# haoheliu/AudioLDM2

Hardware: AMD Instinct MI355X
Metric: audio_seconds_per_second (higher is better)
Workload: dtype f32 storage/accumulate; each product = 6 bf16 MFMA partial products of exact 3-part operand splits (fp32-grade); 1 GPU; audioldm2-full: batch 8 prompts/GPU x 1 GPU, 10.24 s @16 kHz, 200 DDIM steps, CFG 3.5, eta 1.0, n_candidates 1; one step = sample_log + VAE decode + HiFi-GAN + D2H of the waveform; synthetic conditioning, random-init weights, host-CPU RNG noise; global_batch=8, parallelism=prompt-sharded replicas x1, weight_broadcast_bytes=0

## Files before the change

audioldm2_amd/csrc/api.hip:

```cpp
#include "common.h"
#include <string.h>

namespace aldm {
static thread_local char g_err[512] = "";
void set_error(const char* fmt, ...) {
    va_list ap;
    va_start(ap, fmt);
    vsnprintf(g_err, sizeof(g_err), fmt, ap);
    va_end(ap);
}
}

extern "C" int aldm_version(void) { return 11; }
extern "C" const char* aldm_last_error(void) { return aldm::g_err; }
```

audioldm2_amd/csrc/norm.hip:

```cpp
#include <stdlib.h>
#include "igemm_epilogue.h"

namespace aldm {

constexpr int GN_ITERS = 16;
constexpr int GN_UNROLL = 8;

struct GnPart {
    float n, mean, m2;
};

__device__ __forceinline__ void gn_merge(double& n, double& mean, double& m2, double nb, double mb, double m2b) {
    if (nb <= 0.0) return;
    const double nt = n + nb;
    const double dlt = mb - mean;
    mean += dlt * (nb / nt);
    m2 += m2b + dlt * dlt * (n * nb / nt);
    n = nt;
}

template <bool FUSED>
__global__ __launch_bounds__(256) void gn_partial_kernel(const float* __restrict__ x1,
                                                         const float* __restrict__ x2, int P,
                                                         int C1, int C2, int G, int cols, int rows,
                                                         int chunk_px, float* __restrict__ ws, float eps,
                                                         const float* __restrict__ gamma,
                                                         const float* __restrict__ beta,
                                                         float* __restrict__ scale, float* __restrict__ shift, int gpb,
                                                         char* __restrict__ dst = nullptr, char* __restrict__ dst_raw = nullptr,
                                                         int parts = 3, int act = ALDM_ACT_NONE, int raw_parts = 3,
                                                         float f16_scale = 0.f) {
    const int C = C1 + C2;
    const int Cg4 = (C / G) >> 2;
    const int b = blockIdx.y;
    const int chunk = FUSED ? 0 : blockIdx.x;
    const int g_lo = FUSED ? blockIdx.x * gpb : 0;
    const int c4_lo = g_lo * Cg4, C4 = c4_lo + gpb * Cg4;
    const int p0 = chunk * chunk_px;
    const int p1 = min(P, p0 + chunk_px);
    const int tid = threadIdx.x;
    const int tx = tid % cols, ty = tid / cols;
    __shared__ GnPart ps[256];
    const int npass = (C4 - c4_lo + cols - 1) / cols;
    __shared__ double gacc[64][3];
    if (tid < 64) gacc[tid][0] = gacc[tid][1] = gacc[tid][2] = 0.0;
    __syncthreads();
    for (int cp = 0; cp < npass; ++cp) {
        const int c4 = c4_lo + cp * cols + tx;
        GnPart part = {0.f, 0.f, 0.f};
        if (ty < rows && c4 < C4 && p0 + ty < p1) {
            const int c = c4 << 2;
            const bool first = c < C1;
            const float* src = first ? x1 + (int64_t)b * P * C1 + c : x2 + (int64_t)b * P * C2 + (c - C1);
            const int pitch = first ? C1 : C2;
            float sa[GN_UNROLL], sq[GN_UNROLL];
#pragma unroll
            for (int u = 0; u < GN_UNROLL; ++u) sa[u] = sq[u] = 0.f;
            int p = p0 + ty;
            const float pivot = src[(int64_t)p * pitch];
            int cnt = 0;
            for (; p + (GN_UNROLL - 1) * rows < p1; p += GN_UNROLL * rows) {
                f32x4 v[GN_UNROLL];
#pragma unroll
                for (int u = 0; u < GN_UNROLL; ++u)
                    v[u] = *reinterpret_cast<const f32x4*>(src + (int64_t)(p + u * rows) * pitch) - pivot;
#pragma unroll
                for (int u = 0; u < GN_UNROLL; ++u) {
                    sa[u] += (v[u][0] + v[u][1]) + (v[u][2] + v[u][3]);
                    sq[u] += (v[u][0] * v[u][0] + v[u][1] * v[u][1]) + (v[u][2] * v[u][2] + v[u][3] * v[u][3]);
                }
                cnt += GN_UNROLL;
            }
            for (; p < p1; p += rows) {
                const f32x4 v = *reinterpret_cast<const f32x4*>(src + (int64_t)p * pitch) - pivot;
                sa[0] += (v[0] + v[1]) + (v[2] + v[3]);
                sq[0] += (v[0] * v[0] + v[1] * v[1]) + (v[2] * v[2] + v[3] * v[3]);
                ++cnt;
            }
            float s = 0.f, ss = 0.f;
#pragma unroll
            for (int u = 0; u < GN_UNROLL; u += 2) {
                s += sa[u] + sa[u + 1];
                ss += sq[u] + sq[u + 1];
            }
            const float n = 4.0f * (float)cnt;
            const float md = s / n;
            part.n = n;
            part.mean = pivot + md;
            part.m2 = fmaxf(ss - s * md, 0.f);
        }
        if constexpr (FUSED) {
            __shared__ double wred[4][3];
            const int mygl = (c4 - c4_lo) / Cg4;
            for (int gl = 0; gl < gpb; ++gl) {
                const bool mine = part.n > 0.f && mygl == gl;
                double n = mine ? (double)part.n : 0.0, mean = mine ? (double)part.mean : 0.0, m2 = mine ? (double)part.m2 : 0.0;
#pragma unroll
                for (int o = 32; o > 0; o >>= 1) {
                    const double nb = __shfl_xor(n, o), mb = __shfl_xor(mean, o), m2b = __shfl_xor(m2, o);
                    gn_merge(n, mean, m2, nb, mb, m2b);
                }
                if ((tid & 63) == 0) {
                    wred[tid >> 6][0] = n;
                    wred[tid >> 6][1] = mean;
                    wred[tid >> 6][2] = m2;
                }
                __syncthreads();
                if (tid == 0) {
                    double an = gacc[gl][0], am = gacc[gl][1], a2 = gacc[gl][2];
                    for (int w = 0; w < 4; ++w) gn_merge(an, am, a2, wred[w][0], wred[w][1], wred[w][2]);
                    gacc[gl][0] = an;
                    gacc[gl][1] = am;
                    gacc[gl][2] = a2;
                }
                __syncthreads();
            }
            continue;
        }
        ps[tid] = part;
        __syncthreads();
        if (tid < gpb) {
            const int g = g_lo + tid;
            const int base = c4_lo + cp * cols;
            const int lo = max(g * Cg4, base), hi = min((g + 1) * Cg4, min(C4, base + cols));
            if (lo < hi) {
                double n = gacc[tid][0], mean = gacc[tid][1], m2 = gacc[tid][2];
                for (int yy = 0; yy < rows; ++yy)
                    for (int cc = lo; cc < hi; ++cc) {
                        const GnPart& t = ps[yy * cols + (cc - base)];
                        gn_merge(n, mean, m2, (double)t.n, (double)t.mean, (double)t.m2);
                    }
                gacc[tid][0] = n;
                gacc[tid][1] = mean;
                gacc[tid][2] = m2;
            }
        }
        __syncthreads();
    }
    if (FUSED) {
        const int Cg = C / G;
        __shared__ float fin[64][2];
        if (tid < gpb) {
            const double n = gacc[tid][0];
            double var = n > 0.0 ? gacc[tid][2] / n : 0.0;
            if (var < 0.0) var = 0.0;
            fin[tid][0] = (float)gacc[tid][1];
            fin[tid][1] = (float)(1.0 / sqrt(var + (double)eps));
        }
        __syncthreads();
        __shared__ float lsc[256], lsh[256];
        for (int c = g_lo * Cg + tid; c < (g_lo + gpb) * Cg; c += 256) {
            const int g = c / Cg - g_lo;
            const float sc = fin[g][1] * (gamma ? gamma[c] : 1.f);
            const float sh = (beta ? beta[c] : 0.f) - fin[g][0] * sc;
            scale[(int64_t)b * C + c] = sc;
            shift[(int64_t)b * C + c] = sh;
            if (dst) {
                lsc[c - g_lo * Cg] = sc;
                lsh[c - g_lo * Cg] = sh;
            }
        }
        if (dst) {
            __syncthreads();
            const int c_lo = g_lo * Cg, sw = (gpb * Cg) >> 3;
            for (int i = tid; i < P * sw; i += 256) {
                const int p = i / sw;
                const int cl = (i - p * sw) << 3;
                const int c = c_lo + cl;
                const int64_t row = (int64_t)b * P + p;
                const float* src = c < C1 ? x1 + row * C1 + c : x2 + row * C2 + (c - C1);
                f32x4 v0 = *reinterpret_cast<const f32x4*>(src);
                f32x4 v1 = *reinterpret_cast<const f32x4*>(src + 4);
                const int64_t off = (row * (C >> 5) + (c >> 5)) * (64 * parts) + (c & 31) * 2;
                u32x2 p0[3], p1[3];
                if (dst_raw) {
                    const int64_t roff = (row * (C >> 5) + (c >> 5)) * (64 * raw_parts) + (c & 31) * 2;
                    split4_parts(v0, p0, raw_parts);
                    split4_parts(v1, p1, raw_parts);
#pragma unroll
                    for (int q = 0; q < 3; ++q)
                        if (q < raw_parts)
                            *reinterpret_cast<u32x4*>(dst_raw + roff + q * 64) = u32x4{p0[q][0], p0[q][1], p1[q][0], p1[q][1]};
                }
#pragma unroll
                for (int e = 0; e < 4; ++e) {
                    v0[e] = __builtin_fmaf(v0[e], lsc[cl + e], lsh[cl + e]);
                    v1[e] = __builtin_fmaf(v1[e], lsc[cl + 4 + e], lsh[cl + 4 + e]);
                }
                if (act == ALDM_ACT_SILU) {
#pragma unroll
                    for (int e = 0; e < 4; ++e) {
                        v0[e] = silu_fast(v0[e]);
                        v1[e] = silu_fast(v1[e]);
                    }
                }
                split4_fmt(v0, p0, parts, f16_scale);
                split4_fmt(v1, p1, parts, f16_scale);
#pragma unroll
                for (int q = 0; q < 3; ++q)
                    if (q < parts) *reinterpret_cast<u32x4*>(dst + off + q * 64) = u32x4{p0[q][0], p0[q][1], p1[q][0], p1[q][1]};
            }
        }
    } else if (tid < G) {
        double* w = reinterpret_cast<double*>(ws) + ((int64_t)(b * gridDim.x + chunk) * G + tid) * 3;
        w[0] = gacc[tid][0];
        w[1] = gacc[tid][1];
        w[2] = gacc[tid][2];
    }
}

__global__ __launch_bounds__(256) void gn_finalize_kernel(const float* __restrict__ ws, int chunks,
                                                          int P, int C, int G, float eps,
                                                          const float* __restrict__ gamma,
                                                          const float* __restrict__ beta,
                                                          float* __restrict__ scale,
                                                          float* __restrict__ shift) {
    const int b = blockIdx.x;
    __shared__ float s_mean[64], s_rstd[64];
    __shared__ double s_part[256][3];
    const int Cg = C / G;
    const double* wsd = reinterpret_cast<const double*>(ws);
    const int LPG = 256 / G >= 1 ? 256 / G : 1;
    {
        const int g = threadIdx.x / LPG, l = threadIdx.x % LPG;
        double n = 0.0, mean = 0.0, m2 = 0.0;
        if (g < G) {
            for (int ch = l; ch < chunks; ch += LPG) {
                const double* w = wsd + ((int64_t)(b * chunks + ch) * G + g) * 3;
                gn_merge(n, mean, m2, w[0], w[1], w[2]);
            }
        }
        s_part[threadIdx.x][0] = n;
        s_part[threadIdx.x][1] = mean;
        s_part[threadIdx.x][2] = m2;
    }
    __syncthreads();
    if (threadIdx.x < G) {
        const int g = threadIdx.x;
        double n = 0.0, mean = 0.0, m2 = 0.0;
        for (int l = 0; l < LPG; ++l) gn_merge(n, mean, m2, s_part[g * LPG + l][0], s_part[g * LPG + l][1], s_part[g * LPG + l][2]);
        double var = n > 0.0 ? m2 / n : 0.0;
        if (var < 0.0) var = 0.0;
        s_mean[g] = (float)mean;
        s_rstd[g] = (float)(1.0 / sqrt(var + (double)eps));
    }
    __syncthreads();
    for (int c = threadIdx.x; c < C; c += blockDim.x) {
        const int g = c / Cg;
        const float ga = gamma ? gamma[c] : 1.f;
        const float be = beta ? beta[c] : 0.f;
        const float sc = s_rstd[g] * ga;
        scale[(int64_t)b * C + c] = sc;
        shift[(int64_t)b * C + c] = be - s_mean[g] * sc;
    }
}

constexpr int LN_MAXV = 8;

template <int MAXV, int R, bool RMS = false>
__global__ __launch_bounds__(256) void layernorm_kernel(const float* __restrict__ x,
                                                        float* __restrict__ y, int M, int C,
                                                        const float* __restrict__ gamma,
                                                        const float* __restrict__ beta, float eps,
                                                        void* __restrict__ y_split, int parts, float f16_scale) {
    const int lane = threadIdx.x & 63;
    const int row0 = (blockIdx.x * 4 + (threadIdx.x >> 6)) * R;
    if (row0 >= M) return;
    const int C4 = C >> 2;
    f32x4 v[R][MAXV];
#pragma unroll
    for (int r = 0; r < R; ++r) {
        const float* xr = x + (int64_t)min(row0 + r, M - 1) * C;
#pragma unroll
        for (int i = 0; i < MAXV; ++i) {
            const int c4 = lane + 64 * i;
            v[r][i] = c4 < C4 ? *reinterpret_cast<const f32x4*>(xr + 4 * c4) : f32x4{0.f, 0.f, 0.f, 0.f};
        }
    }
    f32x4 ga[MAXV], be[MAXV];
#pragma unroll
    for (int i = 0; i < MAXV; ++i) {
        const int c4 = min(lane + 64 * i, C4 - 1);
        ga[i] = *reinterpret_cast<const f32x4*>(gamma + 4 * c4);
        be[i] = RMS ? f32x4{0.f, 0.f, 0.f, 0.f} : *reinterpret_cast<const f32x4*>(beta + 4 * c4);
    }
    float mean[R], rstd[R];
#pragma unroll
    for (int r = 0; r < R; ++r) {
        float s = 0.f;
#pragma unroll
        for (int i = 0; i < MAXV; ++i) s += (v[r][i][0] + v[r][i][1]) + (v[r][i][2] + v[r][i][3]);
#pragma unroll
        for (int o = 32; o > 0; o >>= 1) s += __shfl_xor(s, o);
        mean[r] = RMS ? 0.f : s / (float)C;
    }
#pragma unroll
    for (int r = 0; r < R; ++r) {
        float q = 0.f;
#pragma unroll
        for (int i = 0; i < MAXV; ++i) {
            if (lane + 64 * i < C4) {
                const f32x4 dlt = v[r][i] - mean[r];
                q += (dlt[0] * dlt[0] + dlt[1] * dlt[1]) + (dlt[2] * dlt[2] + dlt[3] * dlt[3]);
            }
        }
#pragma unroll
        for (int o = 32; o > 0; o >>= 1) q += __shfl_xor(q, o);
        rstd[r] = 1.0f / sqrtf(q / (float)C + eps);
    }
#pragma unroll
    for (int r = 0; r < R; ++r) {
        if (row0 + r >= M) break;
        float* yr = y ? y + (int64_t)(row0 + r) * C : nullptr;
#pragma unroll
        for (int i = 0; i < MAXV; ++i) {
            const int c4 = lane + 64 * i;
            if (c4 < C4) {
                const f32x4 o = (v[r][i] - mean[r]) * rstd[r] * ga[i] + be[i];
                if (yr) *reinterpret_cast<f32x4*>(yr + 4 * c4) = o;
                if (y_split) {
                    if (f16_scale != 0.f) {
                        u32x2 part[3];
                        split4_f16(o, f16_scale, part);
                        char* base = reinterpret_cast<char*>(y_split) + ((int64_t)(row0 + r) * (C >> 5) + (c4 >> 3)) * 128 + (c4 & 7) * 8;
                        *reinterpret_cast<u32x2*>(base) = part[0];
                        *reinterpret_cast<u32x2*>(base + 64) = part[1];
                    } else {
                        split_store4(y_split, row0 + r, C, 4 * c4, o, parts);
                    }
                }
            }
        }
    }
}

template <bool MASKED, bool BIASED = false>
__global__ __launch_bounds__(256) void softmax_rows_kernel(const float* __restrict__ x,
                                                           float* __restrict__ y, int N,
                                                           float scale, const float* __restrict__ keymask,
                                                           int rows_per_batch, int q_rows, int q_pos0,
                                                           const float* __restrict__ bias = nullptr) {
    extern __shared__ __attribute__((aligned(16))) float srow[];
    __shared__ float red[4];
    const int64_t row = blockIdx.x;
    const float* xr = x + row * N;
    float* yr = y + row * N;
    const int tid = threadIdx.x;
    float mx = -INFINITY;
    const float* km = nullptr;
    int jmax = N;
    const float* br = nullptr;
    if (MASKED) {
        km = keymask + (row / rows_per_batch) * N;
        jmax = BIASED ? N : q_pos0 + (int)(row % q_rows) + 1;
    }
    if (BIASED) br = bias + (row % rows_per_batch) * N;
    for (int i = tid; i < N; i += 256) {
        float v = xr[i] * scale;
        if (BIASED) v += br[i];
        if (MASKED && (i >= jmax || km[i] == 0.0f)) v = -INFINITY;
        srow[i] = v;
        mx = fmaxf(mx, v);
    }
#pragma unroll
    for (int o = 32; o > 0; o >>= 1) mx = fmaxf(mx, __shfl_xor(mx, o));
    if ((tid & 63) == 0) red[tid >> 6] = mx;
    __syncthreads();
    mx = fmaxf(fmaxf(red[0], red[1]), fmaxf(red[2], red[3]));
    __syncthreads();
    float s = 0.f;
    for (int i = tid; i < N; i += 256) {
        const float e = (MASKED && srow[i] == -INFINITY) ? 0.0f : expf(srow[i] - mx);
        srow[i] = e;
        s += e;
    }
#pragma unroll
    for (int o = 32; o > 0; o >>= 1) s += __shfl_xor(s, o);
    if ((tid & 63) == 0) red[tid >> 6] = s;
    __syncthreads();
    s = (red[0] + red[1]) + (red[2] + red[3]);
    const float inv = 1.0f / s;
    for (int i = tid; i < N; i += 256) yr[i] = srow[i] * inv;
}

static void gn_geometry(int P, int C, int* cols, int* rows, int* chunk_px, int* chunks) {
    const int C4 = C / 4;
    *cols = C4 < 256 ? C4 : 256;
    *rows = 256 / *cols;
    if (*rows < 1) *rows = 1;
    *chunk_px = *rows * GN_ITERS;
    *chunks = (P + *chunk_px - 1) / *chunk_px;
}

}

using namespace aldm;

extern "C" int64_t aldm_gn_ws_floats(int B, int P, int C, int G) {
    int cols, rows, chunk_px, chunks;
    gn_geometry(P, C, &cols, &rows, &chunk_px, &chunks);
    return (int64_t)B * chunks * G * 6 + 2;
}

extern "C" int aldm_split_rows(const float* x1, const float* x2, int C1, int C2, int64_t rows, int P, const float* scale,
                               const float* shift, int act, void* dst, void* dst_raw, int parts, void* stream);
extern "C" int aldm_split_rows_f16(const float* x1, const float* x2, int C1, int C2, int64_t rows, int P, const float* scale,
                                   const float* shift, int act, float slope, void* dst, void* dst_raw, int raw_parts, float f16_scale,
                                   void* stream);

static int groupnorm_launch(const float* x1, const float* x2, int B, int P, int C1, int C2, int G, float eps,
                            const float* gamma, const float* beta, float* scale, float* shift, float* ws, void* dst,
                            void* dst_raw, int parts, int act, void* stream, int raw_parts = 0, float f16_scale = 0.f) {
    if (raw_parts == 0) raw_parts = parts;
    if (!x2) C2 = 0;
    const int C = C1 + C2;
    ALDM_CHECK(x1 && scale && shift && ws, "aldm_groupnorm_stats: null pointer");
    ws = reinterpret_cast<float*>((reinterpret_cast<uintptr_t>(ws) + 7) & ~uintptr_t(7));
    ALDM_CHECK(G > 0 && G <= 64 && C % G == 0 && (C / G) % 4 == 0 && C1 % 4 == 0,
               "aldm_groupnorm_stats: need C%%G==0, (C/G)%%4==0, C1%%4==0 (C1=%d C2=%d G=%d)", C1, C2, G);
    int cols, rows, chunk_px, chunks;
    gn_geometry(P, C, &cols, &rows, &chunk_px, &chunks);
    hipStream_t st = (hipStream_t)stream;
    static const int64_t fused_max = [] {
        const char* e = getenv("ALDM_GN_FUSED_MAX");
        return e ? (int64_t)atoll(e) : (int64_t)1 << 17;
    }();
    int gs = 1;
    while (gs < G && gs * B < 256 && G % (gs * 2) == 0) gs *= 2;
    const int gpb = G / gs;
    if ((int64_t)P * C <= fused_max && P <= 1024 && gpb <= 4) {
        const int c4b = gpb * (C / G) / 4;
        const int fcols = c4b < 256 ? c4b : 256, frows = 256 / fcols;
        const int slab = gpb * (C / G);
        static const bool fuse_split = [] {
            const char* e = getenv("ALDM_GN_SPLIT_FUSED");
            return e == nullptr || e[0] != '0';
        }();
        if (dst && fuse_split && slab % 8 == 0 && slab <= 256 && C1 % 8 == 0) {
            hipLaunchKernelGGL(gn_partial_kernel<true>, dim3(gs, B), dim3(256), 0, st, x1, x2, P, C1, C2, G, fcols, frows, P, ws,
                               eps, gamma, beta, scale, shift, gpb, reinterpret_cast<char*>(dst),
                               reinterpret_cast<char*>(dst_raw), parts, act, raw_parts, f16_scale);
            ALDM_LAUNCH_CHECK("aldm_groupnorm_split");
            return 0;
        }
        hipLaunchKernelGGL(gn_partial_kernel<true>, dim3(gs, B), dim3(256), 0, st, x1, x2, P, C1, C2, G, fcols,
                           frows, P, ws, eps, gamma, beta, scale, shift, gpb, nullptr, nullptr, 3, ALDM_ACT_NONE);
    } else {
        hipLaunchKernelGGL(gn_partial_kernel<false>, dim3(chunks, B), dim3(256), 0, st, x1, x2, P, C1, C2, G,
                           cols, rows, chunk_px, ws, eps, gamma, beta, scale, shift, G);
        hipLaunchKernelGGL(gn_finalize_kernel, dim3(B), dim3(256), 0, st, ws, chunks, P, C, G, eps, gamma,
                           beta, scale, shift);
    }
    ALDM_LAUNCH_CHECK("aldm_groupnorm_stats");
    if (dst) {
        if (f16_scale != 0.f)
            return aldm_split_rows_f16(x1, x2, C1, C2, (int64_t)B * P, P, scale, shift, act, 0.f, dst, dst_raw, raw_parts, f16_scale, stream);
        return aldm_split_rows(x1, x2, C1, C2, (int64_t)B * P, P, scale, shift, act, dst, dst_raw, parts, stream);
    }
    return 0;
}

extern "C" int aldm_groupnorm_stats(const float* x1, const float* x2, int B, int P, int C1, int C2,
                                    int G, float eps, const float* gamma, const float* beta,
                                    float* scale, float* shift, float* ws, void* stream) {
    return groupnorm_launch(x1, x2, B, P, C1, C2, G, eps, gamma, beta, scale, shift, ws, nullptr, nullptr, 3, ALDM_ACT_NONE,
                            stream);
}

extern "C" int aldm_groupnorm_split(const float* x1, const float* x2, int B, int P, int C1, int C2, int G, float eps,
                                    const float* gamma, const float* beta, int act, float* scale, float* shift, float* ws,
                                    void* dst, void* dst_raw, int parts, void* stream) {
    if (!x2) C2 = 0;
    ALDM_CHECK(dst != nullptr && (parts == 2 || parts == 3) && (C1 + C2) % 32 == 0 && C1 % 8 == 0 && C2 % 8 == 0,
               "aldm_groupnorm_split: need dst, parts 2|3, (C1+C2) %% 32 == 0, C1 %% 8 == 0 (C1=%d C2=%d)", C1, C2);
    ALDM_CHECK(act == ALDM_ACT_NONE || act == ALDM_ACT_SILU, "aldm_groupnorm_split: activation %d not supported", act);
    ALDM_CHECK(((reinterpret_cast<uintptr_t>(dst) | reinterpret_cast<uintptr_t>(dst_raw)) & 15) == 0,
               "aldm_groupnorm_split: split images must be 16-byte aligned");
    return groupnorm_launch(x1, x2, B, P, C1, C2, G, eps, gamma, beta, scale, shift, ws, dst, dst_raw, parts, act, stream);
}

extern "C" int aldm_groupnorm_split_f16(const float* x1, const float* x2, int B, int P, int C1, int C2, int G, float eps,
                                        const float* gamma, const float* beta, int act, float* scale, float* shift, float* ws,
                                        void* dst, void* dst_raw, int raw_parts, float f16_scale, void* stream) {
    if (!x2) C2 = 0;
    ALDM_CHECK(dst != nullptr && f16_scale > 0.0f && (raw_parts == 2 || raw_parts == 3) && (C1 + C2) % 32 == 0 && C1 % 8 == 0 && C2 % 8 == 0,
               "aldm_groupnorm_split_f16: need dst, f16_scale > 0, raw_parts 2|3, (C1+C2) %% 32 == 0, C1 %% 8 == 0 (C1=%d C2=%d)", C1, C2);
    ALDM_CHECK(act == ALDM_ACT_NONE || act == ALDM_ACT_SILU, "aldm_groupnorm_split_f16: activation %d not supported", act);
    ALDM_CHECK(((reinterpret_cast<uintptr_t>(dst) | reinterpret_cast<uintptr_t>(dst_raw)) & 15) == 0,
               "aldm_groupnorm_split_f16: split images must be 16-byte aligned");
    return groupnorm_launch(x1, x2, B, P, C1, C2, G, eps, gamma, beta, scale, shift, ws, dst, dst_raw, 2, act, stream, raw_parts, f16_scale);
}

static int layernorm_launch(const float* x, float* y, void* y_split, int parts, int M, int C, const float* gamma,
                            const float* beta, float eps, void* stream, const char* name, bool rms = false, float f16_scale = 0.f) {
    ALDM_CHECK(parts == 2 || parts == 3, "%s: parts must be 2 or 3", name);
    ALDM_CHECK(x && (y || y_split) && gamma && (beta || rms), "%s: null pointer", name);
    ALDM_CHECK(C % 4 == 0 && C <= 256 * LN_MAXV, "%s: C=%d must be a multiple of 4 and <= %d", name, C, 256 * LN_MAXV);
    ALDM_CHECK(y_split == nullptr || (C % 32 == 0 && (reinterpret_cast<uintptr_t>(y_split) & 15) == 0),
               "%s: a split-image output needs C %% 32 == 0 and 16-byte alignment", name);
    hipStream_t st = (hipStream_t)stream;
#define ALDM_LN(V_, R_)                                                                                             \
    do {                                                                                                            \
        if (rms)                                                                                                    \
            hipLaunchKernelGGL((layernorm_kernel<V_, R_, true>), dim3(cdiv(M, 4 * R_)), dim3(256), 0, st, x, y, M, C, \
                               gamma, beta, eps, y_split, parts, f16_scale);                                        \
        else                                                                                                        \
            hipLaunchKernelGGL((layernorm_kernel<V_, R_, false>), dim3(cdiv(M, 4 * R_)), dim3(256), 0, st, x, y, M, \
                               C, gamma, beta, eps, y_split, parts, f16_scale);                                     \
    } while (0)
    const int nv = cdiv(C / 4, 64);
    static const int env_r = [] {
        const char* e = getenv("ALDM_LN_R");
        return e ? atoi(e) : 0;
    }();
    if (nv <= 1) {
        if (env_r == 4) ALDM_LN(1, 4);
        else if (env_r == 2) ALDM_LN(1, 2);
        else ALDM_LN(1, 1);
    } else if (nv <= 2) {
        if (env_r == 4) ALDM_LN(2, 4);
        else if (env_r == 2) ALDM_LN(2, 2);
        else ALDM_LN(2, 1);
    } else if (nv <= 4) ALDM_LN(4, 2);
    else ALDM_LN(8, 1);
#undef ALDM_LN
    ALDM_LAUNCH_CHECK(name);
    return 0;
}

extern "C" int aldm_layernorm(const float* x, float* y, int M, int C, const float* gamma,
                              const float* beta, float eps, void* stream) {
    return layernorm_launch(x, y, nullptr, 3, M, C, gamma, beta, eps, stream, "aldm_layernorm");
}

extern "C" int aldm_layernorm_split(const float* x, float* y, void* y_split, int M, int C, const float* gamma,
                                    const float* beta, float eps, int parts, void* stream) {
    return layernorm_launch(x, y, y_split, parts, M, C, gamma, beta, eps, stream, "aldm_layernorm_split");
}

extern "C" int aldm_layernorm_split_f16(const float* x, float* y, void* y_split, int M, int C, const float* gamma,
                                        const float* beta, float eps, float f16_scale, void* stream) {
    ALDM_CHECK(y_split != nullptr && f16_scale > 0.0f, "aldm_layernorm_split_f16: need y_split and f16_scale > 0");
    return layernorm_launch(x, y, y_split, 2, M, C, gamma, beta, eps, stream, "aldm_layernorm_split_f16", false, f16_scale);
}

extern "C" int aldm_rmsnorm(const float* x, float* y, int M, int C, const float* weight, float eps, void* stream) {
    return layernorm_launch(x, y, nullptr, 3, M, C, weight, nullptr, eps, stream, "aldm_rmsnorm", true);
}

extern "C" int aldm_softmax_rows(const float* x, float* y, int64_t M, int N, float scale,
                                 void* stream) {
    ALDM_CHECK(x && y && M > 0 && N > 0, "aldm_softmax_rows: bad args");
    ALDM_CHECK((int64_t)N * 4 <= 60 * 1024, "aldm_softmax_rows: row of %d floats exceeds the 60 KiB LDS stage", N);
    ALDM_CHECK(M < (1ll << 31), "aldm_softmax_rows: too many rows");
    hipLaunchKernelGGL(softmax_rows_kernel<false>, dim3((unsigned)M), dim3(256), (size_t)N * 4,
                       (hipStream_t)stream, x, y, N, scale, nullptr, 1, 1, 0);
    ALDM_LAUNCH_CHECK("aldm_softmax_rows");
    return 0;
}

extern "C" int aldm_softmax_rows_masked(const float* x, float* y, int B, int heads, int q_rows, int N, float scale,
                                        const float* keymask, int q_pos0, void* stream) {
    ALDM_CHECK(x && y && keymask && B > 0 && heads > 0 && q_rows > 0 && N > 0 && q_pos0 >= 0,
               "aldm_softmax_rows_masked: bad args");
    ALDM_CHECK((int64_t)N * 4 <= 60 * 1024, "aldm_softmax_rows_masked: row of %d floats exceeds the 60 KiB LDS stage", N);
    const int64_t M = (int64_t)B * heads * q_rows;
    ALDM_CHECK(M < (1ll << 31), "aldm_softmax_rows_masked: too many rows");
    hipLaunchKernelGGL(softmax_rows_kernel<true>, dim3((unsigned)M), dim3(256), (size_t)N * 4, (hipStream_t)stream, x, y,
                       N, scale, keymask, heads * q_rows, q_rows, q_pos0);
    ALDM_LAUNCH_CHECK("aldm_softmax_rows_masked");
    return 0;
}

extern "C" int aldm_softmax_rows_bias(const float* x, float* y, int B, int heads, int q_rows, int N, float scale,
                                      const float* bias, const float* keymask, void* stream) {
    ALDM_CHECK(x && y && bias && keymask && B > 0 && heads > 0 && q_rows > 0 && N > 0, "aldm_softmax_rows_bias: bad args");
    ALDM_CHECK((int64_t)N * 4 <= 60 * 1024, "aldm_softmax_rows_bias: row of %d floats exceeds the 60 KiB LDS stage", N);
    const int64_t M = (int64_t)B * heads * q_rows;
    ALDM_CHECK(M < (1ll << 31), "aldm_softmax_rows_bias: too many rows");
    hipLaunchKernelGGL((softmax_rows_kernel<true, true>), dim3((unsigned)M), dim3(256), (size_t)N * 4, (hipStream_t)stream, x,
                       y, N, scale, keymask, heads * q_rows, q_rows, 0, bias);
    ALDM_LAUNCH_CHECK("aldm_softmax_rows_bias");
    return 0;
}
```

audioldm2_amd/lib.py:

```python
from __future__ import annotations

import ctypes as C
import os

_HERE = os.path.dirname(os.path.abspath(__file__))
LIB_PATH = os.environ.get("ALDM_LIB_PATH") or os.path.join(_HERE, "libaldm_hip.so")
ABI_VERSION = 11

ACT_NONE, ACT_SILU, ACT_LRELU, ACT_TANH, ACT_LOGCLAMP, ACT_GELU, ACT_GELU_TANH = range(7)
B_PACKED, B_NT = 0, 1
EPI_PLAIN, EPI_GEGLU, EPI_QKV = 0, 1, 2
FMT_BF16, FMT_F16 = 0, 1


class IgemmDesc(C.Structure):

    _fields_ = [
        ("x1", C.c_void_p), ("x2", C.c_void_p),
        ("C1", C.c_int32), ("C2", C.c_int32),
        ("pix1", C.c_int32), ("pix2", C.c_int32),
        ("B", C.c_int32), ("H", C.c_int32), ("W", C.c_int32),
        ("up_h", C.c_int32), ("up_w", C.c_int32),
        ("KH", C.c_int32), ("KW", C.c_int32), ("SH", C.c_int32), ("SW", C.c_int32),
        ("PH", C.c_int32), ("PW", C.c_int32), ("DH", C.c_int32), ("DW", C.c_int32),
        ("OH", C.c_int32), ("OW", C.c_int32),
        ("pre_scale", C.c_void_p), ("pre_shift", C.c_void_p),
        ("pre_act", C.c_int32), ("pre_slope", C.c_float),
        ("w", C.c_void_p),
        ("b_mode", C.c_int32), ("ldb", C.c_int32),
        ("K", C.c_int32), ("N", C.c_int32),
        ("bias", C.c_void_p), ("rowbias", C.c_void_p), ("res", C.c_void_p), ("out", C.c_void_p),
        ("ldo", C.c_int32), ("act", C.c_int32), ("act_slope", C.c_float), ("alpha", C.c_float),
        ("accumulate", C.c_int32),
        ("out_mul", C.c_int32), ("out_off", C.c_int32), ("out_len", C.c_int32),
        ("batch", C.c_int32),
        ("stride_x", C.c_int64), ("stride_w", C.c_int64), ("stride_o", C.c_int64),
        ("rowbias_ld", C.c_int32), ("epi_mode", C.c_int32),
        ("ws", C.c_void_p), ("ws_floats", C.c_int64),
        ("hint_bm", C.c_int32), ("hint_bn", C.c_int32), ("hint_splits", C.c_int32), ("hint_kgroups", C.c_int32),
        ("w_split", C.c_void_p), ("hint_mma", C.c_int32), ("hint_stages", C.c_int32),
        ("a_split", C.c_void_p), ("out_split", C.c_void_p), ("out_split_c", C.c_int32), ("split_parts", C.c_int32),
        ("out_split_act", C.c_int32), ("out_split_slope", C.c_float),
        ("k_split", C.c_void_p), ("vt_split", C.c_void_p), ("qkv_c", C.c_int32), ("qkv_rows", C.c_int32),
        ("a_fmt", C.c_int32), ("acc_scale", C.c_float), ("out_split_parts", C.c_int32),
        ("out_split_fmt", C.c_int32), ("out_split_scale", C.c_float), ("vt_scale", C.c_float),
    ]


_SIGS = {
    "aldm_version": (C.c_int, []),
    "aldm_last_error": (C.c_char_p, []),
    "aldm_igemm": (C.c_int, [C.POINTER(IgemmDesc), C.c_void_p]),
    "aldm_igemm_plan": (C.c_int, [C.POINTER(IgemmDesc), C.POINTER(C.c_int), C.POINTER(C.c_int),
                                  C.POINTER(C.c_int64), C.POINTER(C.c_int), C.POINTER(C.c_int),
                                  C.POINTER(C.c_int)]),
    "aldm_igemm_ws_floats": (C.c_int64, [C.POINTER(IgemmDesc)]),
    "aldm_igemm_plan_stages": (C.c_int, [C.POINTER(IgemmDesc)]),
    "aldm_igemm_force": (None, [C.c_int, C.c_int, C.c_int, C.c_int]),
    "aldm_igemm_force_stages": (None, [C.c_int]),
    "aldm_igemm_wave8_mask": (C.c_int, [C.c_int]),
    "aldm_split_image_bytes": (C.c_int64, [C.c_int64, C.c_int, C.c_int]),
    "aldm_split_rows": (C.c_int, [C.c_void_p, C.c_void_p, C.c_int, C.c_int, C.c_int64, C.c_int, C.c_void_p, C.c_void_p,
                                  C.c_int, C.c_void_p, C.c_void_p, C.c_int, C.c_void_p]),
    "aldm_split_rows_act": (C.c_int, [C.c_void_p, C.c_void_p, C.c_int, C.c_int, C.c_int64, C.c_int, C.c_void_p, C.c_void_p,
                                      C.c_int, C.c_float, C.c_void_p, C.c_void_p, C.c_int, C.c_void_p]),
    "aldm_layernorm_split": (C.c_int, [C.c_void_p, C.c_void_p, C.c_void_p, C.c_int, C.c_int, C.c_void_p, C.c_void_p,
                                       C.c_float, C.c_int, C.c_void_p]),
    "aldm_attention_d32_split": (C.c_int, [C.c_void_p, C.c_void_p, C.c_void_p, C.c_void_p, C.c_void_p, C.c_int, C.c_int,
                                           C.c_int, C.c_int, C.c_int, C.c_int, C.c_int, C.c_int, C.c_int,
                                           C.c_void_p, C.c_float, C.c_void_p]),
    "aldm_split_bytes_parts": (C.c_int64, [C.c_int, C.c_int, C.c_int]),
    "aldm_pack_split_bf16_parts": (C.c_int, [C.c_void_p, C.c_void_p, C.c_int, C.c_int, C.c_int, C.c_void_p]),
    "aldm_pack_split_f16": (C.c_int, [C.c_void_p, C.c_void_p, C.c_int, C.c_int, C.c_float, C.c_void_p]),
    "aldm_split_rows_f16": (C.c_int, [C.c_void_p, C.c_void_p, C.c_int, C.c_int, C.c_int64, C.c_int, C.c_void_p, C.c_void_p,
                                      C.c_int, C.c_float, C.c_void_p, C.c_void_p, C.c_int, C.c_float, C.c_void_p]),
    "aldm_groupnorm_split_f16": (C.c_int, [C.c_void_p, C.c_void_p, C.c_int, C.c_int, C.c_int, C.c_int, C.c_int, C.c_float,
                                           C.c_void_p, C.c_void_p, C.c_int, C.c_void_p, C.c_void_p, C.c_void_p, C.c_void_p,
                                           C.c_void_p, C.c_int, C.c_float, C.c_void_p]),
    "aldm_layernorm_split_f16": (C.c_int, [C.c_void_p, C.c_void_p, C.c_void_p, C.c_int, C.c_int, C.c_void_p, C.c_void_p,
                                           C.c_float, C.c_float, C.c_void_p]),
    "aldm_igemm_mma": (C.c_int, [C.c_int]),
    "aldm_split_bytes": (C.c_int64, [C.c_int, C.c_int]),
    "aldm_pack_split_bf16": (C.c_int, [C.c_void_p, C.c_void_p, C.c_int, C.c_int, C.c_void_p]),
    "aldm_pack_weight": (C.c_int, [C.c_void_p, C.c_void_p, C.c_int, C.c_int, C.c_int, C.c_int,
                                   C.c_int, C.c_int, C.c_int, C.c_void_p]),
    "aldm_pack_kn": (C.c_int, [C.c_void_p, C.c_void_p, C.c_int, C.c_int, C.c_int, C.c_int,
                               C.c_int64, C.c_int64, C.c_void_p]),
    "aldm_groupnorm_stats": (C.c_int, [C.c_void_p, C.c_void_p, C.c_int, C.c_int, C.c_int, C.c_int,
                                       C.c_int, C.c_float, C.c_void_p, C.c_void_p, C.c_void_p,
                                       C.c_void_p, C.c_void_p, C.c_void_p]),
    "aldm_gn_ws_floats": (C.c_int64, [C.c_int, C.c_int, C.c_int, C.c_int]),
    "aldm_groupnorm_split": (C.c_int, [C.c_void_p, C.c_void_p, C.c_int, C.c_int, C.c_int, C.c_int, C.c_int, C.c_float,
                                       C.c_void_p, C.c_void_p, C.c_int, C.c_void_p, C.c_void_p, C.c_void_p, C.c_void_p,
                                       C.c_void_p, C.c_int, C.c_void_p]),
    "aldm_layernorm": (C.c_int, [C.c_void_p, C.c_void_p, C.c_int, C.c_int, C.c_void_p, C.c_void_p,
                                 C.c_float, C.c_void_p]),
    "aldm_attention_mma": (C.c_int, [C.c_int]),
    "aldm_attention_sched": (C.c_int, [C.c_int]),
    "aldm_attention_d32_presplit_f16": (C.c_int, [C.c_void_p, C.c_void_p, C.c_void_p, C.c_void_p, C.c_void_p, C.c_int, C.c_float,
                                                  C.c_int, C.c_int, C.c_int, C.c_int, C.c_int, C.c_int, C.c_float, C.c_float,
                                                  C.c_float, C.c_float, C.c_void_p]),
    "aldm_attention_d32_presplit": (C.c_int, [C.c_void_p, C.c_void_p, C.c_void_p, C.c_void_p, C.c_void_p, C.c_int, C.c_int,
                                              C.c_int, C.c_int, C.c_int, C.c_int, C.c_int, C.c_float, C.c_void_p]),
    "aldm_vt_regroup": (C.c_int, [C.c_void_p, C.c_void_p, C.c_int, C.c_int, C.c_int, C.c_int, C.c_void_p]),
    "aldm_attention_d32": (C.c_int, [C.c_void_p, C.c_void_p, C.c_void_p, C.c_void_p, C.c_int,
                                     C.c_int, C.c_int, C.c_int, C.c_int, C.c_int, C.c_int, C.c_int,
                                     C.c_void_p, C.c_float, C.c_void_p]),
    "aldm_rel_attention": (C.c_int, [C.c_void_p, C.c_void_p, C.c_void_p, C.c_void_p, C.c_int, C.c_int, C.c_int, C.c_int,
                                     C.c_int, C.c_int, C.c_int, C.c_int, C.c_void_p, C.c_void_p, C.c_int, C.c_void_p,
                                     C.c_void_p]),
    "aldm_rowscale_add": (C.c_int, [C.c_void_p, C.c_void_p, C.c_void_p, C.c_void_p, C.c_int64, C.c_int, C.c_int, C.c_void_p]),
    "aldm_rmsnorm": (C.c_int, [C.c_void_p, C.c_void_p, C.c_int, C.c_int, C.c_void_p, C.c_float, C.c_void_p]),
    "aldm_softmax_rows_bias": (C.c_int, [C.c_void_p, C.c_void_p, C.c_int, C.c_int, C.c_int, C.c_int, C.c_float, C.c_void_p,
                                         C.c_void_p, C.c_void_p]),
    "aldm_resample_sinc": (C.c_int, [C.c_void_p, C.c_void_p, C.c_void_p, C.c_int, C.c_int, C.c_int, C.c_int, C.c_int, C.c_int,
                                     C.c_int, C.c_void_p]),
    "aldm_power_spec": (C.c_int, [C.c_void_p, C.c_void_p, C.c_int64, C.c_int, C.c_int, C.c_int, C.c_void_p]),
    "aldm_col_affine": (C.c_int, [C.c_void_p, C.c_void_p, C.c_void_p, C.c_void_p, C.c_int64, C.c_int, C.c_void_p]),
    "aldm_bicubic_patchify": (C.c_int, [C.c_void_p, C.c_void_p, C.c_int, C.c_int, C.c_int, C.c_int, C.c_int, C.c_void_p]),
    "aldm_token_mean": (C.c_int, [C.c_void_p, C.c_void_p, C.c_int, C.c_int, C.c_int, C.c_void_p]),
    "aldm_row_cosine": (C.c_int, [C.c_void_p, C.c_void_p, C.c_void_p, C.c_int, C.c_int, C.c_float, C.c_void_p]),
    "aldm_decode_linear": (C.c_int, [C.c_void_p, C.c_int, C.c_int, C.c_int, C.c_void_p, C.c_int, C.c_void_p, C.c_void_p,
                                     C.c_void_p, C.c_float, C.c_int, C.c_void_p, C.c_int, C.c_void_p, C.c_int, C.c_void_p]),
    "aldm_decode_attention": (C.c_int, [C.c_void_p, C.c_int, C.c_void_p, C.c_void_p, C.c_void_p, C.c_void_p, C.c_int, C.c_int,
                                        C.c_int, C.c_float, C.c_void_p, C.c_int, C.c_void_p]),
    "aldm_decode_gemv_slices": (C.c_int, [C.c_int, C.c_int]),
    "aldm_decode_gemv": (C.c_int, [C.c_void_p, C.c_int, C.c_int, C.c_int64, C.c_void_p, C.c_int, C.c_int, C.c_int, C.c_void_p,
                                   C.c_int, C.c_void_p, C.c_void_p]),
    "aldm_decode_reduce_ln": (C.c_int, [C.c_void_p, C.c_int, C.c_int64, C.c_int, C.c_void_p, C.c_void_p, C.c_void_p, C.c_int,
                                        C.c_int, C.c_int, C.c_void_p, C.c_int, C.c_void_p, C.c_void_p, C.c_float, C.c_void_p,
                                        C.c_int, C.c_void_p, C.c_int, C.c_void_p]),
    "aldm_decode_attention_parts": (C.c_int, [C.c_void_p, C.c_int, C.c_int, C.c_int64, C.c_void_p, C.c_void_p, C.c_void_p,
                                              C.c_void_p, C.c_void_p, C.c_int, C.c_int, C.c_int, C.c_float, C.c_void_p, C.c_int,
                                              C.c_void_p]),
    "aldm_softmax_rows_masked": (C.c_int, [C.c_void_p, C.c_void_p, C.c_int, C.c_int, C.c_int, C.c_int, C.c_float,
                                           C.c_void_p, C.c_int, C.c_void_p]),
    "aldm_softmax_rows": (C.c_int, [C.c_void_p, C.c_void_p, C.c_int64, C.c_int, C.c_float,
                                    C.c_void_p]),
    "aldm_geglu": (C.c_int, [C.c_void_p, C.c_void_p, C.c_int64, C.c_int, C.c_void_p]),
    "aldm_timestep_embedding": (C.c_int, [C.c_void_p, C.c_void_p, C.c_int, C.c_int, C.c_float,
                                          C.c_void_p]),
    "aldm_nchw_to_nhwc": (C.c_int, [C.c_void_p, C.c_void_p, C.c_int, C.c_int, C.c_int, C.c_int,
                                    C.c_void_p]),
    "aldm_nhwc_to_nchw": (C.c_int, [C.c_void_p, C.c_void_p, C.c_int, C.c_int, C.c_int, C.c_void_p]),
    "aldm_ddim_step": (C.c_int, [C.c_void_p, C.c_void_p, C.c_void_p, C.c_void_p, C.c_void_p,
                                 C.c_void_p, C.c_int64, C.c_void_p]),
    "aldm_ddim_step_indexed": (C.c_int, [C.c_void_p, C.c_void_p, C.c_void_p, C.c_void_p, C.c_void_p, C.c_void_p, C.c_int64,
                                         C.c_int, C.c_void_p]),
    "aldm_plms_first_step": (C.c_int, [C.c_void_p, C.c_void_p, C.c_void_p, C.c_void_p, C.c_void_p, C.c_void_p, C.c_void_p,
                                       C.c_int64, C.c_void_p]),
    "aldm_plms_step_indexed": (C.c_int, [C.c_void_p, C.c_void_p, C.c_void_p, C.c_void_p, C.c_void_p, C.c_void_p, C.c_int64,
                                         C.c_int, C.c_void_p]),
    "aldm_step_advance": (C.c_int, [C.c_void_p, C.c_void_p, C.c_void_p, C.c_int, C.c_int, C.c_void_p]),
    "aldm_ddpm_step": (C.c_int, [C.c_void_p, C.c_void_p, C.c_void_p, C.c_void_p, C.c_void_p, C.c_int64,
                                 C.c_void_p]),
    "aldm_inpaint_blend": (C.c_int, [C.c_void_p, C.c_void_p, C.c_void_p, C.c_void_p, C.c_void_p,
                                     C.c_int64, C.c_void_p]),
    "aldm_axpby": (C.c_int, [C.c_void_p, C.c_void_p, C.c_void_p, C.c_float, C.c_float, C.c_int64,
                             C.c_void_p]),
    "aldm_reflect_pad_1d": (C.c_int, [C.c_void_p, C.c_void_p, C.c_int, C.c_int, C.c_int, C.c_int,
                                      C.c_void_p]),
    "aldm_mag_phase": (C.c_int, [C.c_void_p, C.c_void_p, C.c_void_p, C.c_int64, C.c_int, C.c_int,
                                 C.c_int, C.c_void_p]),
    "aldm_row_l2norm": (C.c_int, [C.c_void_p, C.c_void_p, C.c_int64, C.c_int, C.c_int, C.c_void_p]),
}

EXPORTED_SYMBOLS = tuple(_SIGS.keys())
TEST_HOOK_SIGS = {"aldm_debug_drop_product": (C.c_int, [C.c_int])}
TESTHOOKS_LIB_PATH = os.path.join(_HERE, "libaldm_hip_testhooks.so")

_lib = None


def source_hash(family: str = "all") -> str:
    import glob
    import hashlib
    h = hashlib.sha256()
    files = sorted(glob.glob(os.path.join(_HERE, "csrc", "*.hip")) + glob.glob(os.path.join(_HERE, "csrc", "*.h")) +
                   glob.glob(os.path.join(os.path.dirname(_HERE), "include", "*.h")))
    if family == "igemm":
        files = [f for f in files if os.path.basename(f).startswith("igemm") or os.path.basename(f) in ("common.h", "aldm_hip.h")]
    elif family != "all":
        raise ValueError(f"source_hash: unknown family {family!r}")
    for f in files:
        h.update(os.path.basename(f).encode())
        with open(f, "rb") as fh:
            h.update(fh.read())
    return h.hexdigest()[:16]


def tuning_hash() -> str:
    import glob
    import hashlib
    h = hashlib.sha256()
    for f in sorted(glob.glob(os.path.join(_HERE, "tuning", "*.json"))):
        h.update(os.path.basename(f).encode())
        with open(f, "rb") as fh:
            h.update(fh.read())
    return h.hexdigest()[:16]


def load():
    global _lib
    if _lib is not None:
        return _lib
    if not os.path.exists(LIB_PATH):
        raise RuntimeError(
            f"{LIB_PATH} is missing: the HIP kernel library has not been built. Run "
            "`python -c 'import __graft_entry__ as g; g.build()'` (or `make -C audioldm2_amd/csrc`). "
            "There is no CPU fallback for the sampling hot path."
        )
    lib = C.CDLL(LIB_PATH)
    for name, (res, args) in _SIGS.items():
        fn = getattr(lib, name)
        fn.restype = res
        fn.argtypes = args
    for name, (res, args) in TEST_HOOK_SIGS.items():
        fn = getattr(lib, name, None)
        if fn is not None:
            fn.restype = res
            fn.argtypes = args
    ver = lib.aldm_version()
    if ver != ABI_VERSION:
        raise RuntimeError(f"libaldm_hip.so ABI version {ver} != expected {ABI_VERSION}; rebuild")
    _lib = lib
    return lib


def check(rc: int, what: str = ""):
    if rc != 0:
        msg = load().aldm_last_error().decode("utf-8", "replace")
        raise RuntimeError(f"libaldm_hip {what} failed ({rc}): {msg}")
```

audioldm2_amd/ops.py:

```python
from __future__ import annotations

import ctypes as C
import json
import os
from dataclasses import dataclass
from typing import List, Optional, Sequence, Tuple

import torch

from . import lib as _l
from .lib import (ACT_GELU, ACT_GELU_TANH, ACT_LOGCLAMP, ACT_LRELU, ACT_NONE, ACT_SILU, ACT_TANH, B_NT, B_PACKED,
                  IgemmDesc)


def _stream() -> int:
    return torch.cuda.current_stream().cuda_stream


def _p(t: Optional[torch.Tensor]):
    return None if t is None else t.data_ptr()


def _chk(t: torch.Tensor, name: str):
    if not (t.is_cuda and t.dtype == torch.float32 and t.is_contiguous()):
        raise RuntimeError(f"{name}: expected a contiguous fp32 CUDA tensor, got "
                           f"{t.dtype} {t.device} contiguous={t.is_contiguous()}")


MMA_MODE = os.environ.get("ALDM_MMA", "bf16x6")
MMA_MODES = ("f32", "bf16x6", "bf16x3", "f16x3")
assert MMA_MODE in MMA_MODES, MMA_MODE


def set_mma(mode: str) -> str:
    global MMA_MODE
    assert mode in MMA_MODES, mode
    prev, MMA_MODE = MMA_MODE, mode
    if _l._lib is not None or os.path.exists(_l.LIB_PATH):
        try:
            if "ALDM_ATTN_MMA" not in os.environ:
                _l.load().aldm_attention_mma({"f32": 1, "bf16x6": 2, "bf16x3": 3, "f16x3": 2}[mode])
        except RuntimeError:
            pass
    return prev


def split_parts() -> int:
    return 2 if MMA_MODE == "bf16x3" else 3


def f16_mode() -> bool:
    return MMA_MODE == "f16x3"


F16_FF_OUT = os.environ.get("ALDM_F16_FF_OUT", "1") != "0"
F16_ATTN = os.environ.get("ALDM_F16_ATTN", "1") != "0"
F16_ATTN_OUT = os.environ.get("ALDM_F16_ATTN_OUT", "1") != "0"


F16_GEGLU_MAX_SLACK_LOG2 = 20.0


def _pow2_scale(bound: float) -> float:
    import math
    if not (bound > 0.0) or not math.isfinite(bound):
        return 1.0
    return float(2.0 ** math.floor(math.log2(32768.0 / bound)))


def _absmax_cached(t: Optional[torch.Tensor]) -> float:
    if t is None:
        return 0.0
    c = getattr(t, "_aldm_absmax", None)
    if c is None or c[0] != t._version:
        if torch.cuda.is_current_stream_capturing():
            raise RuntimeError("f16x3: the bound of a normalisation's parameters must be known before graph capture (run one eager step)")
        c = (t._version, float(t.detach().abs().max()))
        try:
            t._aldm_absmax = c
        except (AttributeError, RuntimeError):
            pass
    return c[1]


def _row_norm_bound(gamma: torch.Tensor, beta: Optional[torch.Tensor], C: int) -> float:
    import math
    b2 = 0.0
    if beta is not None:
        c = getattr(beta, "_aldm_norm2", None)
        if c is None or c[0] != beta._version:
            c = (beta._version, float(beta.detach().double().norm()))
            try:
                beta._aldm_norm2 = c
            except (AttributeError, RuntimeError):
                pass
        b2 = c[1]
    return _absmax_cached(gamma) * math.sqrt(float(C)) + b2


def _row_norm_typical(gamma: torch.Tensor, beta: Optional[torch.Tensor]) -> float:
    import math
    c = getattr(gamma, "_aldm_norm2", None)
    if c is None or c[0] != gamma._version:
        if torch.cuda.is_current_stream_capturing():
            raise RuntimeError("f16x3: the norm of a normalisation's parameters must be known before graph capture (run one eager step)")
        c = (gamma._version, float(gamma.detach().double().norm()))
        try:
            gamma._aldm_norm2 = c
        except (AttributeError, RuntimeError):
            pass
    b2 = 0.0 if beta is None else getattr(beta, "_aldm_norm2", (0, 0.0))[1]
    return math.sqrt(c[1] ** 2 + b2 ** 2)


def _norm_f16_scale(gamma: torch.Tensor, beta: Optional[torch.Tensor], n: int) -> float:
    import math
    return _pow2_scale(math.sqrt(float(n)) * _absmax_cached(gamma) + _absmax_cached(beta))


@dataclass
class Packed:
    data: torch.Tensor
    N: int
    Cin: int
    KH: int
    KW: int
    bias: Optional[torch.Tensor] = None
    split: Optional[torch.Tensor] = None
    split2: Optional[torch.Tensor] = None
    split16: Optional[torch.Tensor] = None
    w_scale: float = 0.0
    cmax: Optional[float] = None
    bmax: float = 0.0
    geglu: bool = False
    halves: Optional[tuple] = None

    @property
    def K(self) -> int:
        return self.KH * self.KW * self.Cin

    def out_bound(self, rn: float) -> float:
        if self.cmax is None:
            if torch.cuda.is_current_stream_capturing():
                raise RuntimeError("f16x3: a weight's column norms must be known before graph capture (run one eager step)")
            npad = self.data.numel() // (4 * ((self.K + 3) // 4))
            self.cmax = float(self.data.view(-1, npad, 4).double().pow(2).sum((0, 2)).max().sqrt())
            self.bmax = 0.0 if self.bias is None else float(self.bias.abs().max())
        return rn * self.cmax + self.bmax

    def geglu_bound(self, rn: float, rt: float) -> Tuple[float, float]:
        import math
        assert self.geglu
        if self.halves is None:
            if torch.cuda.is_current_stream_capturing():
                raise RuntimeError("f16x3: a weight's column norms must be known before graph capture (run one eager step)")
            npad = self.data.numel() // (4 * ((self.K + 3) // 4))
            cn = self.data.view(-1, npad, 4).double().pow(2).sum((0, 2)).sqrt()[:self.N].view(-1, 2, 32)
            b = torch.zeros(self.N, device=self.data.device) if self.bias is None else self.bias
            b = b.double().view(-1, 2, 32)
            self.halves = tuple((float(cn[:, j].max()), float(cn[:, j].median()), float(b[:, j].abs().max()),
                                 float(b[:, j].pow(2).mean().sqrt())) for j in range(2))
        bound, typ = 1.0, 1.0
        for cmax, cmed, bmax, brms in self.halves:
            bound *= rn * cmax + bmax
            typ *= math.sqrt(rt * rt * cmed * cmed / self.K + brms * brms)
        return bound, typ

    def split16_ptr(self) -> int:
        if self.split16 is None:
            if torch.cuda.is_current_stream_capturing():
                raise RuntimeError("a weight's fp16 split image must exist before graph capture (run one eager step)")
            lib = _l.load()
            self.w_scale = _pow2_scale(float(self.data.abs().max()))
            self.split16 = torch.empty(lib.aldm_split_bytes_parts(self.K, self.N, 2) // 4, device=self.data.device, dtype=torch.int32)
            _l.check(lib.aldm_pack_split_f16(self.data.data_ptr(), self.split16.data_ptr(), self.K, self.N, self.w_scale, _stream()),
                     "pack_split_f16")
        return self.split16.data_ptr()

    def split_ptr(self, parts: int = 3) -> Optional[int]:
        if MMA_MODE == "f32":
            return None
        if parts == 2:
            if self.split2 is None:
                if torch.cuda.is_current_stream_capturing():
                    raise RuntimeError("a weight's 2-part split image must exist before graph capture (run one eager step)")
                lib = _l.load()
                self.split2 = torch.empty(lib.aldm_split_bytes_parts(self.K, self.N, 2) // 4, device=self.data.device,
                                          dtype=torch.int32)
                _l.check(lib.aldm_pack_split_bf16_parts(self.data.data_ptr(), self.split2.data_ptr(), self.K, self.N, 2,
                                                        _stream()), "pack_split_bf16(2)")
            return self.split2.data_ptr()
        if self.split is None:
            if torch.cuda.is_current_stream_capturing():
                return None
            lib = _l.load()
            self.split = torch.empty(lib.aldm_split_bytes(self.K, self.N) // 4, device=self.data.device,
                                     dtype=torch.int32)
            _l.check(lib.aldm_pack_split_bf16(self.data.data_ptr(), self.split.data_ptr(), self.K, self.N,
                                              _stream()), "pack_split_bf16")
        return self.split.data_ptr()


class SplitT:
    __slots__ = ("data", "shape", "fmt", "scale", "rn", "rt")

    def __init__(self, data: torch.Tensor, shape, fmt: str = "bf16", scale: float = 1.0, rn: float = 0.0, rt: float = 0.0):
        self.data = data
        self.shape = tuple(shape)
        self.fmt = fmt
        self.scale = scale
        self.rn = rn
        self.rt = rt

    @property
    def parts(self) -> int:
        return self.data.shape[2]

    @staticmethod
    def empty(shape, device, parts: Optional[int] = None, f16_scale: float = 0.0) -> "SplitT":
        C_ = shape[-1]
        assert C_ % 32 == 0, f"split image needs C % 32 == 0, got {C_}"
        rows = 1
        for s_ in shape[:-1]:
            rows *= s_
        if f16_scale:
            return SplitT(torch.empty((rows, C_ // 32, 2, 32), device=device, dtype=torch.int16), shape, "f16", f16_scale)
        return SplitT(torch.empty((rows, C_ // 32, parts or split_parts(), 32), device=device, dtype=torch.int16), shape)

    @property
    def C(self) -> int:
        return self.shape[-1]

    @property
    def rows(self) -> int:
        return self.data.shape[0]

    @property
    def device(self):
        return self.data.device

    def data_ptr(self) -> int:
        return self.data.data_ptr()

    def view(self, *shape) -> "SplitT":
        shape = tuple(shape[0]) if len(shape) == 1 and isinstance(shape[0], (tuple, list)) else tuple(shape)
        n = 1
        for s_ in shape:
            n *= abs(s_)
        tot = self.rows * self.C
        shape = tuple(tot // n if s_ == -1 else s_ for s_ in shape)
        assert shape[-1] == self.C, "a split image can only be re-viewed over its row dimensions"
        return SplitT(self.data, shape, self.fmt, self.scale, self.rn, self.rt)

    def float(self) -> torch.Tensor:
        if self.fmt == "f16":
            h = self.data.view(torch.float16).float()
            return ((h[:, :, 0] + h[:, :, 1]) / self.scale).reshape(self.shape)
        parts = (self.data.to(torch.int32) << 16).view(torch.float32)
        acc = parts[:, :, 0] + parts[:, :, 1]
        if self.parts == 3:
            acc = acc + parts[:, :, 2]
        return acc.reshape(self.shape)


DMA_MODE = os.environ.get("ALDM_DMA", "1") != "0"


def set_dma(on: bool) -> bool:
    global DMA_MODE
    prev, DMA_MODE = DMA_MODE, bool(on)
    return prev


def use_dma() -> bool:
    return DMA_MODE and MMA_MODE in ("bf16x6", "bf16x3", "f16x3")


def split_rows(x: torch.Tensor, x2: Optional[torch.Tensor] = None, pre=None, act: int = ACT_NONE,
               want_raw: bool = False, slope: float = 0.0):
    _chk(x, "split_rows.x")
    C1 = x.shape[-1]
    C2 = 0
    if x2 is not None:
        _chk(x2, "split_rows.x2")
        assert x2.shape[:-1] == x.shape[:-1]
        C2 = x2.shape[-1]
    shape = (*x.shape[:-1], C1 + C2)
    rows = x.numel() // C1
    P = rows // x.shape[0]
    dst = SplitT.empty(shape, x.device)
    raw = SplitT.empty(shape, x.device) if want_raw else None
    sc = sh = None
    if pre is not None:
        sc, sh = pre
        assert sc.shape == (x.shape[0], C1 + C2) and sc.is_contiguous() and sh.is_contiguous()
    _l.check(_l.load().aldm_split_rows_act(x.data_ptr(), _p(x2), C1, C2, rows, P, _p(sc), _p(sh), act, slope, dst.data_ptr(),
                                           None if raw is None else raw.data_ptr(), dst.parts, _stream()), "split_rows")
    return (dst, raw) if want_raw else dst


PROFILE = None
ATTN_PROFILE = None


_ws = {}
_ws_retired = []
WS_SLOT = 0


def _workspace(lib, d: IgemmDesc, device) -> None:
    need = lib.aldm_igemm_ws_floats(C.byref(d))
    if need <= 0:
        return
    key = (device.index if device.index is not None else torch.cuda.current_device(), WS_SLOT)
    buf = _ws.get(key)
    if buf is None or buf.numel() < need:
        if torch.cuda.is_current_stream_capturing():
            return
        if buf is not None:
            _ws_retired.append(buf)
        buf = torch.empty(max(need, 8 << 20), device=device, dtype=torch.float32)
        _ws[key] = buf
    d.ws = buf.data_ptr()
    d.ws_floats = buf.numel()


_TUNE_FIELDS = ("B", "H", "W", "C1", "C2", "pix1", "up_h", "up_w", "KH", "KW", "SH", "SW", "PH", "PW", "DH", "DW",
                "OH", "OW", "N", "b_mode", "batch", "epi_mode", "out_mul")
_TUNED = None
TUNE_LOG = None


def tune_key(d: IgemmDesc) -> str:
    return ",".join(str(getattr(d, f)) for f in _TUNE_FIELDS) + f",{_pre_mode(d)}" + \
        (("," + ("dma2" if d.split_parts == 2 else "dma")) if d.a_split else "")


def _tuned_table(bx=False):
    global _TUNED
    if _TUNED is None:
        _TUNED = {False: {}, True: {}, "dma": {}, "dma2": {}}
        if os.environ.get("ALDM_NO_TUNING", "0") != "1":
            for mode, name in ((False, "mi355x_igemm.json"), (True, "mi355x_igemm_bf16x6.json"),
                               ("dma", "mi355x_igemm_dma.json"), ("dma2", "mi355x_igemm_dma_bf16x3.json")):
                path = os.path.join(os.environ.get("ALDM_TUNING_DIR", ""), name)
                if not (os.environ.get("ALDM_TUNING_DIR") and os.path.exists(path)):
                    path = os.path.join(os.path.dirname(os.path.abspath(__file__)), "tuning", name)
                if os.path.exists(path):
                    with open(path) as f:
                        _TUNED[mode] = {k: v[:5] if mode is True else v[:4] for k, v in json.load(f)["entries"].items()}
    return _TUNED[bx]


def _set_split_operand(d: IgemmDesc, x: "SplitT", pw: "Packed", so: Optional["SplitT"] = None) -> None:
    d.a_split = x.data_ptr()
    d.split_parts = x.parts
    if x.fmt == "f16":
        d.a_fmt = _l.FMT_F16
        d.w_split = pw.split16_ptr()
        d.acc_scale = 1.0 / (x.scale * pw.w_scale)
        d.out_split_parts = so.parts if so is not None else 3
    else:
        d.w_split = pw.split_ptr(x.parts)
        if so is not None:
            assert so.parts == x.parts and so.fmt == "bf16"


def _igemm(d: IgemmDesc, what: str, device=None):
    lib = _l.load()
    if d.a_split and d.epi_mode == _l.EPI_QKV:
        d.epi_mode = _l.EPI_PLAIN
        key = tune_key(d)
        d.epi_mode = _l.EPI_QKV
    else:
        key = tune_key(d)
    key_t = key
    if TUNE_LOG is not None:
        TUNE_LOG.append(key)
    if d.a_split:
        hint = _tuned_table("dma2" if d.split_parts == 2 else "dma").get(key_t)
        if hint is not None:
            d.hint_bm, d.hint_bn, d.hint_splits, d.hint_stages = hint[:4]
    else:
        hint = _tuned_table(bool(d.w_split)).get(key)
        if hint is not None:
            d.hint_bm, d.hint_bn, d.hint_splits, d.hint_kgroups = hint[:4]
            d.hint_mma = hint[4] if len(hint) > 4 else 0
    _workspace(lib, d, device if device is not None else torch.device("cuda", torch.cuda.current_device()))
    if PROFILE is None:
        _l.check(lib.aldm_igemm(C.byref(d), _stream()), what)
        return
    bm, bn, fl, sp, kg, mma = C.c_int(), C.c_int(), C.c_int64(), C.c_int(), C.c_int(), C.c_int()
    _l.check(lib.aldm_igemm_plan(C.byref(d), C.byref(bm), C.byref(bn), C.byref(fl), C.byref(sp), C.byref(kg),
                                 C.byref(mma)), what)
    e0 = torch.cuda.Event(enable_timing=True)
    e1 = torch.cuda.Event(enable_timing=True)
    e0.record()
    _l.check(lib.aldm_igemm(C.byref(d), _stream()), what)
    e1.record()
    shape = (d.B * d.OH * d.OW, d.N, d.K, d.KH * d.KW, d.C2, int(bool(d.pre_scale)), d.pre_act, d.batch,
             sp.value * 10 + kg.value, int(bool(d.a_split)), int(bool(d.out)), int(bool(d.out_split)), d.split_parts or 3,
             int(d.epi_mode == _l.EPI_GEGLU), int(bool(d.res)))
    PROFILE.append((what, bm.value, bn.value, fl.value, e0, e1, shape,
                    _kernel_name(d, bm.value, bn.value, kg.value, bool(mma.value))))


def _pre_mode(d: IgemmDesc) -> int:
    if not d.pre_scale and d.pre_act == ACT_NONE:
        return 0
    if d.pre_scale and d.pre_act == ACT_NONE:
        return 1
    if d.pre_scale and d.pre_act == ACT_SILU:
        return 2
    if not d.pre_scale and d.pre_act == ACT_LRELU:
        return 3
    return 4


def _kernel_name(d: IgemmDesc, bm: int, bn: int, kg: int = 1, bx: bool = False) -> str:
    if d.a_split:
        nst = _l.load().aldm_igemm_plan_stages(C.byref(d))
        if nst >= 400:
            w8 = (nst - 400) // 10
            return f"igemm_dma_halo_kernel<{bm}, {bn}, {(nst - 400) % 10}, {4 if (bm == 256 or w8) else 2}, {d.split_parts or 3}>"
        if nst >= 300:
            epi = 1 if d.epi_mode == _l.EPI_GEGLU else (2 if d.epi_mode == _l.EPI_QKV else 0)
            return f"igemm_dma_os_kernel<{d.K // 32}, {nst - 300}, {d.split_parts or 3}, {epi}>"
        if nst >= 200:
            return f"igemm_dma_lw_kernel<{bm}, {bn}, {nst - 200}, {4 if bm == 256 else 2}, {d.split_parts or 3}>"
        if nst >= 100:
            return f"igemm_dma_ws_kernel<{bm}, {bn}, {nst - 100}, {d.split_parts or 3}>"
        return f"igemm_dma_kernel<{bm}, {bn}, {nst}, {4 if bm == 256 else 2}, {d.split_parts or 3}>"
    pre = _pre_mode(d)
    wm, wn = (4, 1) if bn == 32 else (2, 2)
    w8 = _wave8_mask if _wave8_mask >= 0 else int(os.environ.get("ALDM_IGEMM_W8", "1"))
    bit = {(128, 128): 1, (64, 128): 2, (128, 64): 4}.get((bm, bn), 0)
    if kg == 1 and d.epi_mode != _l.EPI_GEGLU and (w8 & bit) and (
            bit == 1 if bx else (pre in (1, 2) or (bit == 1 and (w8 & 8)))):
        wm, wn = (4, 2) if bit == 4 else (2, 4)
    if bx and (bm, bn) == (128, 128) and d.epi_mode == _l.EPI_GEGLU and pre == 0:
        wm, wn = 4, 2
    uni = "true" if pre in (1, 2) and (d.OH * d.OW) % bm == 0 else "false"
    return f"igemm_kernel<{bm}, {bn}, {wm}, {wn}, {pre}, {kg}, {uni}, {'true' if bx else 'false'}>"


def igemm_force(bm: int = 0, bn: int = 0, splits: int = 0, kgroups: int = 0, stages: int = 0) -> None:
    _l.load().aldm_igemm_force(bm, bn, splits, kgroups)
    _l.load().aldm_igemm_force_stages(stages)


def attention_mma(mode: int) -> int:
    return _l.load().aldm_attention_mma(mode)


def attention_sched(sched: int) -> int:
    return _l.load().aldm_attention_sched(sched)


def debug_drop_product(on: bool) -> bool:
    fn = getattr(_l.load(), "aldm_debug_drop_product", None)
    if fn is None:
        raise RuntimeError("aldm_debug_drop_product is a test hook of libaldm_hip_testhooks.so; the release library does not "
                           f"export it (run with ALDM_LIB_PATH={_l.TESTHOOKS_LIB_PATH})")
    return bool(fn(1 if on else 0))


def igemm_mma(mode: int) -> int:
    return _l.load().aldm_igemm_mma(mode)


_wave8_mask = -1


def igemm_wave8(mask: int = -1) -> int:
    global _wave8_mask
    _wave8_mask = mask
    return _l.load().aldm_igemm_wave8_mask(mask)


def _npad(n: int) -> int:
    return (n + 31) // 32 * 32


def pack_conv(weight: torch.Tensor, bias: Optional[torch.Tensor] = None) -> Packed:
    w = weight.detach().to(device="cuda", dtype=torch.float32).contiguous()
    if w.dim() == 2:
        N, Cin, KH, KW = w.shape[0], w.shape[1], 1, 1
    elif w.dim() == 3:
        N, Cin, KH, KW = w.shape[0], w.shape[1], 1, w.shape[2]
    else:
        N, Cin, KH, KW = w.shape
    K = KH * KW * Cin
    dst = torch.empty(((K + 3) // 4) * _npad(N) * 4, device="cuda", dtype=torch.float32)
    lib = _l.load()
    _l.check(lib.aldm_pack_weight(w.data_ptr(), dst.data_ptr(), N, Cin, KH, KW, 0, 0, 1, _stream()),
             "pack_weight")
    b = None if bias is None else bias.detach().to(device="cuda", dtype=torch.float32).contiguous()
    return Packed(dst, N, Cin, KH, KW, b)


def pack_geglu(weight: torch.Tensor, bias: Optional[torch.Tensor]) -> Packed:
    two_inner = weight.shape[0]
    inner = two_inner // 2
    assert weight.dim() == 2 and two_inner % 64 == 0
    g = torch.arange(inner // 32).view(-1, 1, 1)
    j = torch.arange(2).view(1, -1, 1)
    l = torch.arange(32).view(1, 1, -1)
    perm = (j * inner + g * 32 + l).reshape(-1).to(weight.device)
    pw = pack_conv(weight.detach()[perm], None if bias is None else bias.detach()[perm])
    pw.geglu = True
    return pw


def linear_geglu(x, pw: Packed, split_out: Optional[str] = None, gate_act: int = ACT_NONE,
                 out: Optional[torch.Tensor] = None):
    is_split = isinstance(x, SplitT)
    if not is_split:
        _chk(x, "linear_geglu.x")
    shp = x.shape
    M = (x.rows if is_split else x.numel() // shp[-1])
    assert shp[-1] == pw.Cin and pw.KH == 1 and pw.KW == 1 and pw.N % 64 == 0
    oshape = (*shp[:-1], pw.N // 2)
    if split_out == "only":
        assert out is None
    elif out is None:
        out = torch.empty(oshape, device=x.device, dtype=torch.float32)
    else:
        _chk(out, "linear_geglu.out")
        assert out.numel() == M * (pw.N // 2), (out.shape, oshape)
        out = out.view(oshape)
    so = None
    if split_out:
        if is_split and x.fmt == "f16" and x.rn > 0.0 and f16_mode() and F16_FF_OUT:
            if pw.geglu:
                bound, typ = pw.geglu_bound(x.rn, x.rt)
            else:
                bound, typ = pw.out_bound(x.rn) ** 2, 0.0
            if typ <= 0.0 or bound <= typ * 2.0 ** F16_GEGLU_MAX_SLACK_LOG2:
                so = SplitT.empty(oshape, x.device, f16_scale=_pow2_scale(bound))
        if so is None:
            so = SplitT.empty(oshape, x.device)
    d = IgemmDesc()
    if is_split:
        _set_split_operand(d, x, pw, so if (so is None or so.fmt == "bf16") else None)
        if so is not None and so.fmt == "f16":
            d.out_split_fmt = _l.FMT_F16; d.out_split_scale = so.scale
    else:
        d.x1 = x.data_ptr(); d.split_parts = 3
        d.w_split = pw.split_ptr(3)
    if so is not None and not is_split:
        d.split_parts = so.parts
    d.C1 = pw.Cin; d.B = 1; d.H = 1; d.W = M; d.up_h = d.up_w = 1
    d.KH = d.KW = d.SH = d.SW = d.DH = d.DW = 1
    d.OH = 1; d.OW = M
    d.w = pw.data.data_ptr(); d.b_mode = B_PACKED; d.K = pw.K; d.N = pw.N
    d.bias = _p(pw.bias); d.out = _p(out); d.ldo = pw.N // 2; d.alpha = 1.0
    if so is not None:
        d.out_split = so.data_ptr(); d.out_split_c = pw.N // 2
    d.epi_mode = _l.EPI_GEGLU; d.batch = 1
    d.act = gate_act
    _igemm(d, "igemm(geglu)")
    return so if split_out == "only" else ((out, so) if split_out else out)


def linear_qkv(x: "SplitT", pw: Packed, heads: int, rows_per_sample: int):
    assert isinstance(x, SplitT) and pw.KH == 1 and pw.KW == 1 and pw.bias is None
    Cq = heads * 32
    assert pw.N == 3 * Cq and x.shape[-1] == pw.Cin
    M = x.rows
    assert M % rows_per_sample == 0
    Bn = M // rows_per_sample
    ragged = rows_per_sample % 32 != 0
    f16_kv = x.fmt == "f16" and x.rn > 0.0 and f16_mode() and F16_ATTN
    P = 2 if f16_kv else (3 if x.fmt == "f16" else x.parts)
    dev = x.device
    q = torch.empty((*x.shape[:-1], Cq), device=dev, dtype=torch.float32)
    if ragged:
        k_img = torch.empty((M + 31, heads, P, 32), device=dev, dtype=torch.int16)[:M]
        vt_img = torch.empty((Bn, heads, -(-rows_per_sample // 32), P, 32, 32), device=dev, dtype=torch.int16)
        vt_raw = torch.empty((heads, -(-M // 32), P, 32, 32), device=dev, dtype=torch.int16)
    else:
        k_img = torch.empty((M, heads, P, 32), device=dev, dtype=torch.int16)
        vt_img = torch.empty((Bn, heads, rows_per_sample // 32, P, 32, 32), device=dev, dtype=torch.int16)
    d = IgemmDesc()
    _set_split_operand(d, x, pw)
    d.out_split_parts = P
    if f16_kv:
        bound = pw.out_bound(x.rn)
        kv_scale = _pow2_scale(bound)
        q_scale = _pow2_scale(bound * (32 ** -0.5) * 1.4426950408889634)
        d.out_split_fmt = _l.FMT_F16; d.out_split_scale = kv_scale; d.vt_scale = kv_scale
        k_img._aldm_f16 = vt_img._aldm_f16 = (q_scale, kv_scale, kv_scale)
    d.C1 = pw.Cin; d.B = 1; d.H = 1; d.W = M; d.up_h = d.up_w = 1
    d.KH = d.KW = d.SH = d.SW = d.DH = d.DW = 1
    d.OH = 1; d.OW = M
    d.w = pw.data.data_ptr(); d.b_mode = B_PACKED; d.K = pw.K; d.N = pw.N
    d.out = q.data_ptr(); d.ldo = Cq; d.alpha = 1.0
    d.k_split = k_img.data_ptr(); d.vt_split = vt_img.data_ptr(); d.qkv_c = Cq; d.qkv_rows = rows_per_sample
    if ragged:
        d.vt_split = vt_raw.data_ptr(); d.qkv_rows = vt_raw.shape[1] * 32
    d.epi_mode = _l.EPI_QKV; d.batch = 1
    _igemm(d, "igemm(qkv)")
    if ragged:
        _l.check(_l.load().aldm_vt_regroup(vt_raw.data_ptr(), vt_img.data_ptr(), Bn, rows_per_sample, heads, P, _stream()),
                 "vt_regroup")
    return q, k_img, vt_img


def attention_presplit(q: torch.Tensor, k_img: torch.Tensor, vt_img: torch.Tensor, heads: int, *,
                       scale: Optional[float] = None, split_out: Optional[str] = None):
    qp, Lq, ldq = _rowview(q, "attn_pre.q")
    B = q.shape[0]
    Lk = k_img.shape[0] // B
    parts = k_img.shape[2]
    assert q.shape[2] == heads * 32 and k_img.shape[1] == heads and vt_img.shape[0] == B and vt_img.shape[2] == -(-Lk // 32)
    if scale is None:
        scale = 32 ** -0.5
    out = None if split_out == "only" else torch.empty((B, Lq, heads * 32), device=q.device, dtype=torch.float32)
    f16s = getattr(k_img, "_aldm_f16", None) or getattr(vt_img, "_aldm_f16", None)
    if f16s is None and parts == 2 and f16_mode():
        raise RuntimeError("attention_presplit: a 2-part K / V^T image without its fp16 scales in f16x3 mode (the scales are an "
                           "attribute of the tensors linear_qkv returned: pass those, not a view or a clone of them)")
    f16_out = f16s is not None and F16_ATTN_OUT
    so = None
    if split_out:
        so = SplitT.empty((B, Lq, heads * 32), q.device, f16_scale=f16s[2]) if f16_out else \
            SplitT.empty((B, Lq, heads * 32), q.device, 3 if f16s is not None else parts)
    ev = None
    if ATTN_PROFILE is not None:
        ev = (torch.cuda.Event(enable_timing=True), torch.cuda.Event(enable_timing=True))
        ev[0].record()
    if f16s is not None:
        assert abs(scale - 32 ** -0.5) < 1e-12, "the fp16 images' q scale was chosen for the default softmax scale"
        _l.check(_l.load().aldm_attention_d32_presplit_f16(qp, k_img.data_ptr(), vt_img.data_ptr(), _p(out),
                                                           None if so is None else so.data_ptr(),
                                                           3 if so is None else (0 if so.fmt == "f16" else so.parts),
                                                           0.0 if so is None or so.fmt != "f16" else so.scale, B, heads,
                                                           Lq, Lk, ldq, heads * 32, scale, f16s[0], f16s[1], f16s[2], _stream()),
                 "attention_d32_presplit_f16")
    else:
        _l.check(_l.load().aldm_attention_d32_presplit(qp, k_img.data_ptr(), vt_img.data_ptr(), _p(out),
                                                       None if so is None else so.data_ptr(), parts, B, heads, Lq, Lk, ldq,
                                                       heads * 32, scale, _stream()), "attention_d32_presplit")
    if ev is not None:
        ev[1].record()
        ATTN_PROFILE.append((B, heads, Lq, Lk, False, 4.0 * B * heads * Lq * Lk * 32, ev[0], ev[1]))
    if not split_out:
        return out
    return so if split_out == "only" else (out, so)


def pack_convtr1d(weight: torch.Tensor, bias: Optional[torch.Tensor], stride: int) -> List[Packed]:
    w = weight.detach().to(device="cuda", dtype=torch.float32).contiguous()
    Cin, N, KW = w.shape
    T = (KW + stride - 1) // stride
    lib = _l.load()
    b = None if bias is None else bias.detach().to(device="cuda", dtype=torch.float32).contiguous()
    out = []
    for ph in range(stride):
        dst = torch.empty(((T * Cin + 3) // 4) * _npad(N) * 4, device="cuda", dtype=torch.float32)
        _l.check(lib.aldm_pack_weight(w.data_ptr(), dst.data_ptr(), N, Cin, 1, KW, 1, ph, stride,
                                      _stream()), "pack_weight(tr)")
        out.append(Packed(dst, N, Cin, 1, T, b))
    return out


def conv(x: torch.Tensor, pw: Packed, *, stride=(1, 1), pad=(0, 0), dil=(1, 1), up=(1, 1),
         x2: Optional[torch.Tensor] = None, out_hw: Optional[Tuple[int, int]] = None,
         pre: Optional[Tuple[torch.Tensor, torch.Tensor]] = None, pre_act: int = ACT_NONE,
         pre_slope: float = 0.0, bias: Optional[torch.Tensor] = None,
         rowbias: Optional[torch.Tensor] = None, res: Optional[torch.Tensor] = None,
         act: int = ACT_NONE, act_slope: float = 0.0, alpha: float = 1.0,
         out: Optional[torch.Tensor] = None, accumulate: bool = False,
         remap: Optional[Tuple[int, int, int]] = None,
         use_pw_bias: bool = True, split_out: Optional[str] = None, split_act: int = ACT_NONE, split_slope: float = 0.0):
    is_split = isinstance(x, SplitT)
    if is_split:
        assert x2 is None and pre is None and pre_act == ACT_NONE, "a pre-split operand takes no prologue"
    else:
        _chk(x, "conv.x")
    B, H, W, C1 = x.shape
    C2 = 0
    if x2 is not None:
        _chk(x2, "conv.x2")
        assert x2.shape[:3] == x.shape[:3]
        C2 = x2.shape[3]
    assert C1 + C2 == pw.Cin, f"channels {C1}+{C2} != packed Cin {pw.Cin}"
    VH, VW = H * up[0], W * up[1]
    if out_hw is None:
        OH = (VH + 2 * pad[0] - dil[0] * (pw.KH - 1) - 1) // stride[0] + 1
        OW = (VW + 2 * pad[1] - dil[1] * (pw.KW - 1) - 1) // stride[1] + 1
    else:
        OH, OW = out_hw
    N = pw.N
    if remap is not None:
        out_mul, out_off, out_len = remap
        oshape = (B, 1, out_len, N)
    else:
        out_mul = out_off = out_len = 0
        oshape = (B, OH, OW, N)
    if split_out == "only":
        assert out is None and not accumulate
    elif out is None:
        assert not accumulate
        out = torch.empty(oshape, device=x.device, dtype=torch.float32)
    else:
        _chk(out, "conv.out")
        assert out.numel() == oshape[0] * oshape[1] * oshape[2] * oshape[3], (out.shape, oshape)
    so = SplitT.empty(oshape, x.device) if split_out else None
    if bias is None and use_pw_bias:
        bias = pw.bias
    d = IgemmDesc()
    if is_split:
        _set_split_operand(d, x, pw, so)
    else:
        d.x1 = x.data_ptr(); d.split_parts = so.parts if so is not None else 3
    d.x2 = _p(x2)
    d.C1 = C1; d.C2 = C2; d.pix1 = 0; d.pix2 = 0
    d.B = B; d.H = H; d.W = W; d.up_h = up[0]; d.up_w = up[1]
    d.KH = pw.KH; d.KW = pw.KW; d.SH = stride[0]; d.SW = stride[1]
    d.PH = pad[0]; d.PW = pad[1]; d.DH = dil[0]; d.DW = dil[1]
    d.OH = OH; d.OW = OW
    if pre is not None:
        d.pre_scale = pre[0].data_ptr(); d.pre_shift = pre[1].data_ptr()
    d.pre_act = pre_act; d.pre_slope = pre_slope
    d.w = pw.data.data_ptr(); d.b_mode = B_PACKED; d.ldb = 0
    if not is_split:
        d.w_split = pw.split_ptr(3)
    d.K = pw.K; d.N = N
    d.bias = _p(bias); d.rowbias = _p(rowbias); d.res = _p(res); d.out = _p(out)
    if so is not None:
        d.out_split = so.data_ptr(); d.out_split_c = N
        d.out_split_act = split_act; d.out_split_slope = split_slope
    if rowbias is not None:
        if not (rowbias.dim() == 2 and rowbias.stride(1) == 1 and rowbias.shape == (B, N)):
            raise RuntimeError("conv.rowbias: need a [B, N] fp32 view with unit inner stride")
        d.rowbias_ld = rowbias.stride(0)
    d.ldo = N; d.act = act; d.act_slope = act_slope; d.alpha = alpha
    d.accumulate = 1 if accumulate else 0
    d.out_mul = out_mul; d.out_off = out_off; d.out_len = out_len
    d.batch = 1
    _igemm(d, "igemm(conv)")
    if split_out == "only":
        return so
    return (out.view(oshape), so) if split_out else out.view(oshape)


def linear(x, pw: Packed, **kw):
    shp = x.shape
    if isinstance(x, SplitT):
        M = x.rows
        y = conv(x.view(1, 1, M, shp[-1]), pw, **kw)
    else:
        M = x.numel() // shp[-1]
        y = conv(x.reshape(1, 1, M, shp[-1]), pw, **kw)
    oshape = (*shp[:-1], pw.N)
    if isinstance(y, tuple):
        return y[0].view(oshape), y[1].view(oshape)
    return y.view(oshape)


def _view3(t: torch.Tensor, name: str):
    if not (t.is_cuda and t.dtype == torch.float32 and t.dim() == 3 and t.stride(2) == 1):
        raise RuntimeError(f"{name}: need a [Z, R, D] fp32 CUDA view with unit inner stride")
    return t.data_ptr(), t.stride(0), t.stride(1)


def gemm_nt(a: torch.Tensor, bmat: torch.Tensor, *, alpha: float = 1.0,
            out: Optional[torch.Tensor] = None) -> torch.Tensor:
    ap, sa, lda = _view3(a, "gemm_nt.a")
    bp, sb, ldb = _view3(bmat, "gemm_nt.b")
    Z, M, K = a.shape
    Zb, N, Kb = bmat.shape
    assert Z == Zb and K == Kb and K % 4 == 0
    if out is None:
        out = torch.empty((Z, M, N), device=a.device, dtype=torch.float32)
    d = IgemmDesc()
    d.x1 = ap; d.C1 = K; d.pix1 = lda; d.B = 1; d.H = 1; d.W = M; d.up_h = d.up_w = 1
    d.KH = d.KW = d.SH = d.SW = d.DH = d.DW = 1
    d.OH = 1; d.OW = M
    d.w = bp; d.b_mode = B_NT; d.ldb = ldb; d.K = K; d.N = N
    d.out = out.data_ptr(); d.ldo = N; d.alpha = alpha
    d.batch = Z; d.stride_x = sa; d.stride_w = sb; d.stride_o = M * N
    _igemm(d, "igemm(nt)")
    return out


def pack_kn(src: torch.Tensor) -> torch.Tensor:
    sp, ss, lds = _view3(src, "pack_kn.src")
    Z, K, N = src.shape
    per = ((K + 3) // 4) * _npad(N) * 4
    dst = torch.empty((Z, per), device=src.device, dtype=torch.float32)
    _l.check(_l.load().aldm_pack_kn(sp, dst.data_ptr(), K, N, lds, Z, ss, per, _stream()), "pack_kn")
    return dst


def gemm_packed_batched(a: torch.Tensor, bp: torch.Tensor, K: int, N: int, *,
                        out: Optional[torch.Tensor] = None) -> torch.Tensor:
    _chk(a, "gemm_packed.a")
    Z, M, Ka = a.shape
    assert Ka == K and K % 4 == 0
    if out is None:
        out = torch.empty((Z, M, N), device=a.device, dtype=torch.float32)
    d = IgemmDesc()
    d.x1 = a.data_ptr(); d.C1 = K; d.B = 1; d.H = 1; d.W = M; d.up_h = d.up_w = 1
    d.KH = d.KW = d.SH = d.SW = d.DH = d.DW = 1
    d.OH = 1; d.OW = M
    d.w = bp.data_ptr(); d.b_mode = B_PACKED; d.ldb = 0; d.K = K; d.N = N
    d.out = out.data_ptr(); d.ldo = N; d.alpha = 1.0
    d.batch = Z; d.stride_x = M * K; d.stride_w = bp.shape[1]; d.stride_o = M * N
    _igemm(d, "igemm(packed batched)")
    return out


_gn_ws = {}


def gn_stats(x: torch.Tensor, gamma: torch.Tensor, beta: torch.Tensor, *, groups: int = 32,
             eps: float = 1e-5, x2: Optional[torch.Tensor] = None):
    _chk(x, "gn.x")
    B = x.shape[0]
    C1 = x.shape[-1]
    P = x.numel() // (B * C1)
    C2 = 0
    if x2 is not None:
        _chk(x2, "gn.x2")
        C2 = x2.shape[-1]
    Cc = C1 + C2
    lib = _l.load()
    nws = lib.aldm_gn_ws_floats(B, P, Cc, groups)
    ws = torch.empty(nws, device=x.device, dtype=torch.float32)
    ss = torch.empty((2, B, Cc), device=x.device, dtype=torch.float32)
    _l.check(lib.aldm_groupnorm_stats(x.data_ptr(), _p(x2), B, P, C1, C2, groups, eps,
                                      gamma.data_ptr(), beta.data_ptr(), ss[0].data_ptr(),
                                      ss[1].data_ptr(), ws.data_ptr(), _stream()), "groupnorm_stats")
    return ss[0], ss[1]


def gn_split(x: torch.Tensor, gamma: torch.Tensor, beta: torch.Tensor, *, groups: int = 32, eps: float = 1e-5,
             x2: Optional[torch.Tensor] = None, act: int = ACT_NONE, want_raw: bool = False):
    _chk(x, "gn_split.x")
    B = x.shape[0]
    C1 = x.shape[-1]
    P = x.numel() // (B * C1)
    C2 = 0
    if x2 is not None:
        _chk(x2, "gn_split.x2")
        assert x2.shape[:-1] == x.shape[:-1]
        C2 = x2.shape[-1]
    Cc = C1 + C2
    lib = _l.load()
    ws = torch.empty(lib.aldm_gn_ws_floats(B, P, Cc, groups), device=x.device, dtype=torch.float32)
    ss = torch.empty((2, B, Cc), device=x.device, dtype=torch.float32)
    shape = (*x.shape[:-1], Cc)
    raw = SplitT.empty(shape, x.device) if want_raw else None
    if f16_mode():
        dst = SplitT.empty(shape, x.device, f16_scale=_norm_f16_scale(gamma, beta, (Cc // groups) * P))
        _l.check(lib.aldm_groupnorm_split_f16(x.data_ptr(), _p(x2), B, P, C1, C2, groups, eps, gamma.data_ptr(), beta.data_ptr(), act,
                                              ss[0].data_ptr(), ss[1].data_ptr(), ws.data_ptr(), dst.data_ptr(),
                                              None if raw is None else raw.data_ptr(), 3, dst.scale, _stream()), "groupnorm_split_f16")
        return (dst, raw) if want_raw else dst
    dst = SplitT.empty(shape, x.device)
    _l.check(lib.aldm_groupnorm_split(x.data_ptr(), _p(x2), B, P, C1, C2, groups, eps, gamma.data_ptr(), beta.data_ptr(), act,
                                      ss[0].data_ptr(), ss[1].data_ptr(), ws.data_ptr(), dst.data_ptr(),
                                      None if raw is None else raw.data_ptr(), dst.parts, _stream()), "groupnorm_split")
    return (dst, raw) if want_raw else dst


def layernorm(x: torch.Tensor, gamma: torch.Tensor, beta: torch.Tensor, eps: float = 1e-5,
              split_out: Optional[str] = None):
    _chk(x, "ln.x")
    Cc = x.shape[-1]
    M = x.numel() // Cc
    y = None if split_out == "only" else torch.empty_like(x)
    if not split_out:
        _l.check(_l.load().aldm_layernorm(x.data_ptr(), y.data_ptr(), M, Cc, gamma.data_ptr(),
                                          beta.data_ptr(), eps, _stream()), "layernorm")
        return y
    if f16_mode():
        so = SplitT.empty(x.shape, x.device, f16_scale=_norm_f16_scale(gamma, beta, Cc))
        so.rn = _row_norm_bound(gamma, beta, Cc)
        so.rt = _row_norm_typical(gamma, beta)
        _l.check(_l.load().aldm_layernorm_split_f16(x.data_ptr(), _p(y), so.data_ptr(), M, Cc, gamma.data_ptr(), beta.data_ptr(), eps,
                                                    so.scale, _stream()), "layernorm_split_f16")
        return so if split_out == "only" else (y, so)
    so = SplitT.empty(x.shape, x.device)
    _l.check(_l.load().aldm_layernorm_split(x.data_ptr(), _p(y), so.data_ptr(), M, Cc, gamma.data_ptr(),
                                            beta.data_ptr(), eps, so.parts, _stream()), "layernorm_split")
    return so if split_out == "only" else (y, so)


def _rowview(t: torch.Tensor, name: str):
    if not (t.is_cuda and t.dtype == torch.float32 and t.dim() == 3 and t.stride(2) == 1
            and t.stride(0) == t.shape[1] * t.stride(1)):
        raise RuntimeError(f"{name}: need [B, L, D] fp32 CUDA view with unit inner stride")
    return t.data_ptr(), t.shape[1], t.stride(1)


def attention(q: torch.Tensor, k: torch.Tensor, v: torch.Tensor, heads: int, *,
              mask: Optional[torch.Tensor] = None, scale: Optional[float] = None,
              split_out: Optional[str] = None):
    qp, Lq, ldq = _rowview(q, "attn.q")
    kp, Lk, ldk = _rowview(k, "attn.k")
    vp, Lv, ldv = _rowview(v, "attn.v")
    assert Lk == Lv and q.shape[2] == heads * 32
    B = q.shape[0]
    if scale is None:
        scale = 32 ** -0.5
    out = None if split_out == "only" else torch.empty((B, Lq, heads * 32), device=q.device, dtype=torch.float32)
    if mask is not None:
        mask = mask.to(torch.float32).reshape(B, Lk).contiguous()
    ev = None
    if ATTN_PROFILE is not None:
        ev = (torch.cuda.Event(enable_timing=True), torch.cuda.Event(enable_timing=True))
        ev[0].record()
    if not split_out:
        _l.check(_l.load().aldm_attention_d32(qp, kp, vp, out.data_ptr(), B, heads, Lq, Lk, ldq, ldk, ldv,
                                              heads * 32, _p(mask), scale, _stream()), "attention_d32")
        res = out
    else:
        so = SplitT.empty((B, Lq, heads * 32), q.device)
        _l.check(_l.load().aldm_attention_d32_split(qp, kp, vp, _p(out), so.data_ptr(), so.parts, B, heads, Lq, Lk, ldq,
                                                    ldk, ldv, heads * 32, _p(mask), scale, _stream()), "attention_d32_split")
        res = so if split_out == "only" else (out, so)
    if ev is not None:
        ev[1].record()
        ATTN_PROFILE.append((B, heads, Lq, Lk, mask is not None, 4.0 * B * heads * Lq * Lk * 32, ev[0], ev[1]))
    return res


def rmsnorm(x: torch.Tensor, weight: torch.Tensor, eps: float = 1e-6) -> torch.Tensor:
    _chk(x, "rmsnorm.x")
    Cc = x.shape[-1]
    y = torch.empty_like(x)
    _l.check(_l.load().aldm_rmsnorm(x.data_ptr(), y.data_ptr(), x.numel() // Cc, Cc, weight.data_ptr(), eps, _stream()),
             "rmsnorm")
    return y


def softmax_rows_bias(x: torch.Tensor, bias: torch.Tensor, keymask: torch.Tensor, scale: float = 1.0) -> torch.Tensor:
    _chk(x, "softmax_bias.x"); _chk(bias, "softmax_bias.bias"); _chk(keymask, "softmax_bias.keymask")
    B, heads, q_rows, N = x.shape
    assert bias.shape == (heads, q_rows, N) and keymask.shape == (B, N)
    y = torch.empty_like(x)
    _l.check(_l.load().aldm_softmax_rows_bias(x.data_ptr(), y.data_ptr(), B, heads, q_rows, N, scale, bias.data_ptr(),
                                              keymask.data_ptr(), _stream()), "softmax_rows_bias")
    return y


def rel_attention(q: torch.Tensor, k: torch.Tensor, v: torch.Tensor, heads: int, emb_k: torch.Tensor, emb_v: torch.Tensor,
                  mask: torch.Tensor) -> torch.Tensor:
    qp, T, ldq = _rowview(q, "rel_attn.q")
    kp, Tk, ldk = _rowview(k, "rel_attn.k")
    vp, Tv, ldv = _rowview(v, "rel_attn.v")
    B = q.shape[0]
    d = q.shape[2] // heads
    assert T == Tk == Tv and emb_k.shape == emb_v.shape and emb_k.shape[1] == d and emb_k.shape[0] % 2 == 1
    _chk(emb_k, "rel_attn.emb_k"); _chk(emb_v, "rel_attn.emb_v"); _chk(mask, "rel_attn.mask")
    assert mask.shape == (B, T)
    out = torch.empty((B, T, heads * d), device=q.device, dtype=torch.float32)
    _l.check(_l.load().aldm_rel_attention(qp, kp, vp, out.data_ptr(), B, heads, T, d, ldq, ldk, ldv, heads * d,
                                          emb_k.data_ptr(), emb_v.data_ptr(), emb_k.shape[0] // 2, mask.data_ptr(),
                                          _stream()), "rel_attention")
    return out


def rowscale_add(x: torch.Tensor, s: torch.Tensor, res: Optional[torch.Tensor] = None, divide: bool = False) -> torch.Tensor:
    _chk(x, "rowscale.x"); _chk(s, "rowscale.s")
    Cc = x.shape[-1]
    rows = x.numel() // Cc
    assert s.numel() == rows
    if res is not None:
        _chk(res, "rowscale.res")
        assert res.shape == x.shape
    y = torch.empty_like(x)
    _l.check(_l.load().aldm_rowscale_add(x.data_ptr(), s.data_ptr(), _p(res), y.data_ptr(), rows, Cc, 1 if divide else 0,
                                         _stream()), "rowscale_add")
    return y


def resample_sinc(x: torch.Tensor, kernel: torch.Tensor, down: int, up: int, width: int, out_len: int) -> torch.Tensor:
    _chk(x, "resample.x"); _chk(kernel, "resample.kernel")
    B, T = x.shape
    assert kernel.shape[0] == up
    y = torch.empty((B, out_len), device=x.device, dtype=torch.float32)
    _l.check(_l.load().aldm_resample_sinc(x.data_ptr(), kernel.data_ptr(), y.data_ptr(), B, T, out_len, down, up,
                                          kernel.shape[1], width, _stream()), "resample_sinc")
    return y


def power_spec(spec: torch.Tensor, F: int, ld_out: int) -> torch.Tensor:
    _chk(spec, "power_spec.spec")
    M = spec.numel() // spec.shape[-1]
    out = torch.empty((M, ld_out), device=spec.device, dtype=torch.float32)
    _l.check(_l.load().aldm_power_spec(spec.data_ptr(), out.data_ptr(), M, F, spec.shape[-1], ld_out, _stream()),
             "power_spec")
    return out


def col_affine(x: torch.Tensor, scale: torch.Tensor, shift: torch.Tensor) -> torch.Tensor:
    _chk(x, "col_affine.x"); _chk(scale, "col_affine.scale"); _chk(shift, "col_affine.shift")
    Cc = x.shape[-1]
    assert scale.numel() == Cc and shift.numel() == Cc
    y = torch.empty_like(x)
    _l.check(_l.load().aldm_col_affine(x.data_ptr(), scale.data_ptr(), shift.data_ptr(), y.data_ptr(), x.numel() // Cc, Cc,
                                       _stream()), "col_affine")
    return y


def bicubic_patchify(x: torch.Tensor, S: int, p: int) -> torch.Tensor:
    _chk(x, "bicubic_patchify.x")
    B, T, Fm = x.shape
    out = torch.empty((B, (S // p) ** 2, p * p), device=x.device, dtype=torch.float32)
    _l.check(_l.load().aldm_bicubic_patchify(x.data_ptr(), out.data_ptr(), B, T, Fm, S, p, _stream()), "bicubic_patchify")
    return out


def token_mean(x: torch.Tensor) -> torch.Tensor:
    _chk(x, "token_mean.x")
    B, L, Cc = x.shape
    y = torch.empty((B, Cc), device=x.device, dtype=torch.float32)
    _l.check(_l.load().aldm_token_mean(x.data_ptr(), y.data_ptr(), B, L, Cc, _stream()), "token_mean")
    return y


def row_cosine(a: torch.Tensor, b: torch.Tensor, eps: float = 1e-8) -> torch.Tensor:
    _chk(a, "row_cosine.a"); _chk(b, "row_cosine.b")
    assert a.shape == b.shape and a.dim() == 2
    out = torch.empty((a.shape[0],), device=a.device, dtype=torch.float32)
    _l.check(_l.load().aldm_row_cosine(a.data_ptr(), b.data_ptr(), out.data_ptr(), a.shape[0], a.shape[1], eps, _stream()),
             "row_cosine")
    return out


def softmax_rows(x: torch.Tensor, scale: float = 1.0) -> torch.Tensor:
    _chk(x, "softmax.x")
    N = x.shape[-1]
    y = torch.empty_like(x)
    _l.check(_l.load().aldm_softmax_rows(x.data_ptr(), y.data_ptr(), x.numel() // N, N, scale,
                                         _stream()), "softmax_rows")
    return y


def softmax_rows_masked(x: torch.Tensor, keymask: torch.Tensor, q_pos0: int, scale: float = 1.0) -> torch.Tensor:
    _chk(x, "softmax_masked.x")
    _chk(keymask, "softmax_masked.keymask")
    B, heads, q_rows, N = x.shape
    assert keymask.shape == (B, N)
    y = torch.empty_like(x)
    _l.check(_l.load().aldm_softmax_rows_masked(x.data_ptr(), y.data_ptr(), B, heads, q_rows, N, scale,
                                                keymask.data_ptr(), q_pos0, _stream()), "softmax_rows_masked")
    return y


DECODE_MAX_ROWS = 16


def decode_linear(x: torch.Tensor, w_kn: torch.Tensor, bias: Optional[torch.Tensor] = None, *,
                  ln: Optional[Tuple[torch.Tensor, torch.Tensor, float]] = None, act: int = ACT_NONE,
                  res: Optional[torch.Tensor] = None) -> torch.Tensor:
    _chk(x, "decode_linear.x"); _chk(w_kn, "decode_linear.w")
    M, K = x.shape
    assert w_kn.dim() == 2 and w_kn.shape[0] == K and 1 <= M <= DECODE_MAX_ROWS
    N = w_kn.shape[1]
    if res is not None:
        _chk(res, "decode_linear.res")
        assert res.shape == (M, N)
    y = torch.empty((M, N), device=x.device, dtype=torch.float32)
    g, b, eps = ln if ln is not None else (None, None, 0.0)
    if bias is not None:
        _chk(bias, "decode_linear.bias")
        assert bias.numel() == N, f"decode_linear: bias has {bias.numel()} entries for N = {N}"
    for t, nm in ((g, "ln gamma"), (b, "ln beta")):
        if t is not None:
            _chk(t, "decode_linear." + nm)
            assert t.numel() == K, f"decode_linear: {nm} has {t.numel()} entries for K = {K}"
    assert (g is None) == (b is None), "decode_linear: LayerNorm gamma and beta come together"
    _l.check(_l.load().aldm_decode_linear(x.data_ptr(), K, M, K, w_kn.data_ptr(), N, _p(bias), _p(g), _p(b), float(eps), act,
                                          _p(res), N, y.data_ptr(), N, _stream()), "decode_linear")
    return y


def decode_attention(qkv: torch.Tensor, pos: torch.Tensor, k_cache: torch.Tensor, v_cache: torch.Tensor,
                     keymask: torch.Tensor, heads: int, scale: Optional[float] = None) -> torch.Tensor:
    _chk(qkv, "decode_attention.qkv"); _chk(k_cache, "decode_attention.k_cache"); _chk(v_cache, "decode_attention.v_cache")
    _chk(keymask, "decode_attention.keymask")
    B = qkv.shape[0]
    E = heads * 64
    n_tot = keymask.shape[1]
    assert qkv.shape == (B, 3 * E) and keymask.shape[0] == B
    assert k_cache.shape == (B * heads, n_tot, 64) and v_cache.shape == k_cache.shape
    assert pos.is_cuda and pos.dtype == torch.int64 and pos.numel() == 1
    out = torch.empty((B, E), device=qkv.device, dtype=torch.float32)
    _l.check(_l.load().aldm_decode_attention(qkv.data_ptr(), 3 * E, pos.data_ptr(), k_cache.data_ptr(), v_cache.data_ptr(),
                                             keymask.data_ptr(), B, heads, n_tot, 0.125 if scale is None else float(scale),
                                             out.data_ptr(), E, _stream()), "decode_attention")
    return out


def decode_gemv(x: torch.Tensor, w_kn: torch.Tensor, *, xbias: Optional[torch.Tensor] = None, xact: int = ACT_NONE) -> torch.Tensor:
    _chk(x, "decode_gemv.x"); _chk(w_kn, "decode_gemv.w")
    P = 1 if x.dim() == 2 else x.shape[0]
    M, K = x.shape[-2], x.shape[-1]
    assert w_kn.dim() == 2 and w_kn.shape[0] == K and 1 <= M <= DECODE_MAX_ROWS
    N = w_kn.shape[1]
    lib = _l.load()
    S = lib.aldm_decode_gemv_slices(K, N)
    assert S > 0, f"decode_gemv: K = {K} cannot be sliced"
    if xbias is not None:
        _chk(xbias, "decode_gemv.xbias")
        assert xbias.numel() == K
    y = torch.empty((S, M, N), device=x.device, dtype=torch.float32)
    _l.check(lib.aldm_decode_gemv(x.data_ptr(), K, P, M * K, _p(xbias), xact, M, K, w_kn.data_ptr(), N, y.data_ptr(), _stream()),
             "decode_gemv")
    return y


def decode_reduce_ln(part: Optional[torch.Tensor], *, bias: Optional[torch.Tensor] = None, bias_row: Optional[torch.Tensor] = None,
                     res: Optional[torch.Tensor] = None, ln: Optional[Tuple[torch.Tensor, torch.Tensor, float]] = None,
                     want_h: bool = True, xn_out: Optional[torch.Tensor] = None):
    src = part if part is not None else res
    M, N = src.shape[-2], src.shape[-1]
    if part is not None:
        _chk(part, "decode_reduce_ln.part")
        assert part.dim() == 3
    for t, nm in ((bias, "bias"), (res, "res")):
        if t is not None:
            _chk(t, "decode_reduce_ln." + nm)
    if res is not None:
        assert res.shape == (M, N)
    if bias_row is not None:
        assert bias_row.is_cuda and bias_row.dtype == torch.int64 and bias_row.numel() == 1 and bias is not None and bias.dim() == 2
    elif bias is not None:
        assert bias.numel() == N
    dev = src.device
    h = torch.empty((M, N), device=dev, dtype=torch.float32) if want_h else None
    g, b, eps = ln if ln is not None else (None, None, 0.0)
    xn = torch.empty((M, N), device=dev, dtype=torch.float32) if ln is not None else None
    ldn2 = 0
    if xn_out is not None:
        assert ln is not None and xn_out.is_cuda and xn_out.dtype == torch.float32 and xn_out.shape == (M, N) and xn_out.stride(1) == 1
        ldn2 = xn_out.stride(0)
    _l.check(_l.load().aldm_decode_reduce_ln(_p(part), 0 if part is None else part.shape[0], M * N, N, _p(bias), _p(bias_row),
                                             _p(res), N, M, N, _p(h), N, _p(g), _p(b), float(eps), _p(xn), N, _p(xn_out), ldn2,
                                             _stream()), "decode_reduce_ln")
    if ln is None:
        return h
    return (h, xn) if want_h else xn


def decode_attention_parts(qkv_part: torch.Tensor, qbias: Optional[torch.Tensor], pos: torch.Tensor, k_cache: torch.Tensor,
                           v_cache: torch.Tensor, keymask: torch.Tensor, heads: int, scale: Optional[float] = None) -> torch.Tensor:
    _chk(qkv_part, "decode_attention_parts.qkv"); _chk(k_cache, "decode_attention_parts.k_cache")
    _chk(v_cache, "decode_attention_parts.v_cache"); _chk(keymask, "decode_attention_parts.keymask")
    S, B = qkv_part.shape[0], qkv_part.shape[1]
    E = heads * 64
    n_tot = keymask.shape[1]
    assert qkv_part.shape == (S, B, 3 * E) and keymask.shape[0] == B
    assert k_cache.shape == (B * heads, n_tot, 64) and v_cache.shape == k_cache.shape
    assert pos.is_cuda and pos.dtype == torch.int64 and pos.numel() == 1
    if qbias is not None:
        _chk(qbias, "decode_attention_parts.qbias")
        assert qbias.numel() == 3 * E
    out = torch.empty((B, E), device=qkv_part.device, dtype=torch.float32)
    _l.check(_l.load().aldm_decode_attention_parts(qkv_part.data_ptr(), 3 * E, S, B * 3 * E, _p(qbias), pos.data_ptr(),
                                                   k_cache.data_ptr(), v_cache.data_ptr(), keymask.data_ptr(), B, heads, n_tot,
                                                   0.125 if scale is None else float(scale), out.data_ptr(), E, _stream()),
             "decode_attention_parts")
    return out


def geglu(x: torch.Tensor) -> torch.Tensor:
    _chk(x, "geglu.x")
    C2 = x.shape[-1]
    M = x.numel() // C2
    y = torch.empty((*x.shape[:-1], C2 // 2), device=x.device, dtype=torch.float32)
    _l.check(_l.load().aldm_geglu(x.data_ptr(), y.data_ptr(), M, C2 // 2, _stream()), "geglu")
    return y


def timestep_embedding(t: torch.Tensor, dim: int, max_period: float = 10000.0) -> torch.Tensor:
    t = t.to(torch.float32).contiguous()
    out = torch.empty((t.shape[0], dim), device=t.device, dtype=torch.float32)
    _l.check(_l.load().aldm_timestep_embedding(t.data_ptr(), out.data_ptr(), t.shape[0], dim,
                                               max_period, _stream()), "timestep_embedding")
    return out


def nchw_to_nhwc(x: torch.Tensor, rep: int = 1) -> torch.Tensor:
    _chk(x, "nchw_to_nhwc.x")
    B, Cc, H, W = x.shape
    y = torch.empty((rep * B, H, W, Cc), device=x.device, dtype=torch.float32)
    _l.check(_l.load().aldm_nchw_to_nhwc(x.data_ptr(), y.data_ptr(), B, Cc, H * W, rep, _stream()),
             "nchw_to_nhwc")
    return y


def nhwc_to_nchw(x: torch.Tensor) -> torch.Tensor:
    _chk(x, "nhwc_to_nchw.x")
    B, H, W, Cc = x.shape
    y = torch.empty((B, Cc, H, W), device=x.device, dtype=torch.float32)
    _l.check(_l.load().aldm_nhwc_to_nchw(x.data_ptr(), y.data_ptr(), B, Cc, H * W, _stream()),
             "nhwc_to_nchw")
    return y


def ddim_step(x: torch.Tensor, eps: torch.Tensor, noise: torch.Tensor, coef: torch.Tensor,
              x_prev: Optional[torch.Tensor] = None, pred_x0: Optional[torch.Tensor] = None):
    for t, n in ((x, "x"), (eps, "eps"), (noise, "noise"), (coef, "coef")):
        _chk(t, "ddim." + n)
    if x_prev is None:
        x_prev = torch.empty_like(x)
    if pred_x0 is None:
        pred_x0 = torch.empty_like(x)
    _l.check(_l.load().aldm_ddim_step(x.data_ptr(), eps.data_ptr(), noise.data_ptr(), coef.data_ptr(),
                                      x_prev.data_ptr(), pred_x0.data_ptr(), x.numel(), _stream()),
             "ddim_step")
    return x_prev, pred_x0


def ddim_step_indexed(x: torch.Tensor, eps: torch.Tensor, noise_tab: torch.Tensor, coef_tab: torch.Tensor,
                      step_idx: torch.Tensor, pred_x0: Optional[torch.Tensor] = None) -> torch.Tensor:
    for t, n in ((x, "x"), (eps, "eps"), (noise_tab, "noise_tab"), (coef_tab, "coef_tab")):
        _chk(t, "ddim_indexed." + n)
    assert step_idx.dtype == torch.int32 and step_idx.is_cuda and noise_tab.shape[1:] == x.shape and coef_tab.dim() == 2
    assert noise_tab.shape[0] == coef_tab.shape[0]
    _l.check(_l.load().aldm_ddim_step_indexed(x.data_ptr(), eps.data_ptr(), noise_tab.data_ptr(), coef_tab.data_ptr(),
                                              step_idx.data_ptr(), _p(pred_x0), x.numel(), coef_tab.shape[1], _stream()),
             "ddim_step_indexed")
    return x


def plms_first_step(x: torch.Tensor, e_t: torch.Tensor, e_next: Optional[torch.Tensor], coef: torch.Tensor,
                    x_out: Optional[torch.Tensor] = None, pred_x0: Optional[torch.Tensor] = None,
                    hist: Optional[torch.Tensor] = None):
    for t, n in ((x, "x"), (e_t, "e_t"), (coef, "coef")):
        _chk(t, "plms_first." + n)
    assert coef.numel() >= 7 and e_t.numel() in (x.numel(), 2 * x.numel())
    if e_next is not None:
        _chk(e_next, "plms_first.e_next"); _chk(hist, "plms_first.hist")
        assert e_next.shape == e_t.shape and tuple(hist.shape) == (3,) + tuple(x.shape)
    if x_out is None:
        x_out = torch.empty_like(x)
    if pred_x0 is None:
        pred_x0 = torch.empty_like(x)
    _chk(x_out, "plms_first.x_out"); _chk(pred_x0, "plms_first.pred_x0")
    assert x_out.shape == x.shape == pred_x0.shape
    _l.check(_l.load().aldm_plms_first_step(x.data_ptr(), e_t.data_ptr(), _p(e_next), coef.data_ptr(), x_out.data_ptr(),
                                            pred_x0.data_ptr(), _p(hist if e_next is not None else None), x.numel(),
                                            _stream()), "plms_first_step")
    return x_out, pred_x0


def plms_step_indexed(x: torch.Tensor, eps: torch.Tensor, hist: torch.Tensor, coef_tab: torch.Tensor,
                      step_idx: torch.Tensor, pred_x0: Optional[torch.Tensor] = None) -> torch.Tensor:
    for t, n in ((x, "x"), (eps, "eps"), (hist, "hist"), (coef_tab, "coef_tab")):
        _chk(t, "plms_indexed." + n)
    assert step_idx.dtype == torch.int32 and step_idx.is_cuda and coef_tab.dim() == 2
    assert tuple(hist.shape) == (3,) + tuple(x.shape) and eps.numel() in (x.numel(), 2 * x.numel())
    if pred_x0 is not None:
        _chk(pred_x0, "plms_indexed.pred_x0")
        assert pred_x0.shape == x.shape
    _l.check(_l.load().aldm_plms_step_indexed(x.data_ptr(), eps.data_ptr(), hist.data_ptr(), coef_tab.data_ptr(),
                                              step_idx.data_ptr(), _p(pred_x0), x.numel(), coef_tab.shape[1], _stream()),
             "plms_step_indexed")
    return x


def step_advance(step_idx: torch.Tensor, t_tab: torch.Tensor, t_cur: torch.Tensor) -> None:
    _chk(t_tab, "step_advance.t_tab"); _chk(t_cur, "step_advance.t_cur")
    assert step_idx.dtype == torch.int32 and t_tab.dim() == 2 and t_tab.shape[1] == t_cur.numel()
    _l.check(_l.load().aldm_step_advance(step_idx.data_ptr(), t_tab.data_ptr(), t_cur.data_ptr(), t_tab.shape[1],
                                         t_tab.shape[0], _stream()), "step_advance")


def ddpm_step(x: torch.Tensor, eps: torch.Tensor, noise: torch.Tensor, coef: torch.Tensor,
              x_prev: Optional[torch.Tensor] = None) -> torch.Tensor:
    for t, n in ((x, "x"), (eps, "eps"), (noise, "noise"), (coef, "coef")):
        _chk(t, "ddpm." + n)
    if x_prev is None:
        x_prev = torch.empty_like(x)
    _l.check(_l.load().aldm_ddpm_step(x.data_ptr(), eps.data_ptr(), noise.data_ptr(), coef.data_ptr(),
                                      x_prev.data_ptr(), x.numel(), _stream()), "ddpm_step")
    return x_prev


def inpaint_blend(x: torch.Tensor, x0: torch.Tensor, qnoise: torch.Tensor, mask: torch.Tensor,
                  coef: torch.Tensor) -> torch.Tensor:
    for t, n in ((x, "x"), (x0, "x0"), (qnoise, "qnoise"), (mask, "mask"), (coef, "coef")):
        _chk(t, "inpaint." + n)
    assert x.shape == x0.shape == qnoise.shape == mask.shape
    _l.check(_l.load().aldm_inpaint_blend(x0.data_ptr(), qnoise.data_ptr(), mask.data_ptr(),
                                          coef.data_ptr(), x.data_ptr(), x.numel(), _stream()),
             "inpaint_blend")
    return x


def axpby(a: torch.Tensor, b: Optional[torch.Tensor], alpha: float, beta: float = 0.0,
          out: Optional[torch.Tensor] = None) -> torch.Tensor:
    _chk(a, "axpby.a")
    if out is None:
        out = torch.empty_like(a)
    _l.check(_l.load().aldm_axpby(a.data_ptr(), _p(b), out.data_ptr(), alpha, beta, a.numel(),
                                  _stream()), "axpby")
    return out


def reflect_pad_1d(x: torch.Tensor, pad: int) -> torch.Tensor:
    _chk(x, "reflect_pad.x")
    B, T = x.shape
    pitch = (T + 2 * pad + 3) // 4 * 4
    buf = torch.zeros((B, pitch), device=x.device, dtype=torch.float32)
    _l.check(_l.load().aldm_reflect_pad_1d(x.data_ptr(), buf.data_ptr(), B, T, pad, pitch, _stream()),
             "reflect_pad_1d")
    return buf


def frames_gemm(sig: torch.Tensor, frames: int, hop: int, pw: Packed) -> torch.Tensor:
    _chk(sig, "frames_gemm.sig")
    B, pitch = sig.shape
    K = pw.K
    assert K % 4 == 0 and hop % 4 == 0 and (frames - 1) * hop + K <= pitch
    out = torch.empty((B, frames, pw.N), device=sig.device, dtype=torch.float32)
    d = IgemmDesc()
    d.x1 = sig.data_ptr(); d.C1 = K; d.pix1 = hop; d.B = 1; d.H = 1; d.W = frames
    d.up_h = d.up_w = 1
    d.KH = d.KW = d.SH = d.SW = d.DH = d.DW = 1
    d.OH = 1; d.OW = frames
    d.w = pw.data.data_ptr(); d.b_mode = B_PACKED; d.K = K; d.N = pw.N
    d.out = out.data_ptr(); d.ldo = pw.N; d.alpha = 1.0
    d.batch = B; d.stride_x = pitch; d.stride_w = 0; d.stride_o = frames * pw.N
    _igemm(d, "igemm(frames)")
    return out


def mag_phase(spec: torch.Tensor, F: int, ld_mag: int, want_phase: bool = True):
    _chk(spec, "mag_phase.spec")
    M = spec.numel() // spec.shape[-1]
    mag = torch.empty((M, ld_mag), device=spec.device, dtype=torch.float32)
    phase = torch.empty((M, F), device=spec.device, dtype=torch.float32) if want_phase else None
    _l.check(_l.load().aldm_mag_phase(spec.data_ptr(), mag.data_ptr(), _p(phase), M, F,
                                      spec.shape[-1], ld_mag, _stream()), "mag_phase")
    return mag, phase


def row_l2norm(x: torch.Tensor, F: int) -> torch.Tensor:
    _chk(x, "row_l2norm.x")
    M, ld = x.shape
    out = torch.empty((M,), device=x.device, dtype=torch.float32)
    _l.check(_l.load().aldm_row_l2norm(x.data_ptr(), out.data_ptr(), M, F, ld, _stream()), "row_l2norm")
    return out
```

audioldm2_amd/unet.py:

```python
from __future__ import annotations

from typing import List, Optional

import torch
import torch.nn as nn

import os

from . import ops
from .ops import ACT_NONE, ACT_SILU

PRESPLIT_ATTENTION = os.environ.get("ALDM_ATTN_PRESPLIT", "1") != "0" and "ALDM_ATTN_MMA" not in os.environ


class ResBlock(nn.Module):

    def __init__(self, channels, emb_channels, dropout, out_channels=None):
        super().__init__()
        self.channels = channels
        self.out_channels = out_channels or channels
        self.in_layers = nn.Sequential(nn.GroupNorm(32, channels), nn.SiLU(),
                                       nn.Conv2d(channels, self.out_channels, 3, padding=1))
        self.emb_layers = nn.Sequential(nn.SiLU(), nn.Linear(emb_channels, self.out_channels))
        self.out_layers = nn.Sequential(nn.GroupNorm(32, self.out_channels), nn.SiLU(), nn.Dropout(p=dropout),
                                        nn.Conv2d(self.out_channels, self.out_channels, 3, padding=1))
        if self.out_channels == channels:
            self.skip_connection = nn.Identity()
        else:
            self.skip_connection = nn.Conv2d(channels, self.out_channels, 1)
        self._pk = None

    def _prepare(self):
        if self._pk is None:
            c1, c2 = self.in_layers[2], self.out_layers[3]
            self._pk = dict(
                gn1=(self.in_layers[0].weight.detach().float().cuda().contiguous(),
                     self.in_layers[0].bias.detach().float().cuda().contiguous()),
                gn2=(self.out_layers[0].weight.detach().float().cuda().contiguous(),
                     self.out_layers[0].bias.detach().float().cuda().contiguous()),
                conv1=ops.pack_conv(c1.weight, c1.bias),
                conv2=ops.pack_conv(c2.weight, c2.bias),
                skip=None if isinstance(self.skip_connection, nn.Identity)
                else ops.pack_conv(self.skip_connection.weight, self.skip_connection.bias),
            )
        return self._pk

    def run(self, x, e, x2=None):
        pk = self._prepare()
        c2 = 0 if x2 is None else x2.shape[-1]
        if ops.use_dma() and self.channels % 32 == 0 and x.shape[-1] % 8 == 0 and c2 % 8 == 0:
            if pk["skip"] is None:
                assert x2 is None
                a1, skip = ops.gn_split(x, *pk["gn1"], groups=32, eps=1e-5, act=ACT_SILU), x
            else:
                a1, araw = ops.gn_split(x, *pk["gn1"], groups=32, eps=1e-5, x2=x2, act=ACT_SILU, want_raw=True)
                skip = ops.conv(araw, pk["skip"])
            h = ops.conv(a1, pk["conv1"], pad=(1, 1), rowbias=e)
            a2 = ops.gn_split(h, *pk["gn2"], groups=32, eps=1e-5, act=ACT_SILU)
            return ops.conv(a2, pk["conv2"], pad=(1, 1), res=skip)
        sc, sh = ops.gn_stats(x, *pk["gn1"], groups=32, eps=1e-5, x2=x2)
        h = ops.conv(x, pk["conv1"], x2=x2, pad=(1, 1), pre=(sc, sh), pre_act=ACT_SILU, rowbias=e)
        sc2, sh2 = ops.gn_stats(h, *pk["gn2"], groups=32, eps=1e-5)
        if pk["skip"] is None:
            assert x2 is None
            skip = x
        else:
            skip = ops.conv(x, pk["skip"], x2=x2)
        return ops.conv(h, pk["conv2"], pad=(1, 1), pre=(sc2, sh2), pre_act=ACT_SILU, res=skip)


class Downsample(nn.Module):

    def __init__(self, channels, use_conv=True, dims=2, out_channels=None, padding=1):
        super().__init__()
        assert use_conv and dims == 2
        self.channels = channels
        self.out_channels = out_channels or channels
        self.op = nn.Conv2d(channels, self.out_channels, 3, stride=2, padding=padding)
        self._pk = None

    def run(self, x):
        if self._pk is None:
            self._pk = ops.pack_conv(self.op.weight, self.op.bias)
        if ops.use_dma() and self.channels % 32 == 0:
            x = ops.split_rows(x)
        return ops.conv(x, self._pk, stride=(2, 2), pad=(1, 1))


class Upsample(nn.Module):

    def __init__(self, channels, use_conv=True, dims=2, out_channels=None, padding=1):
        super().__init__()
        assert use_conv and dims == 2
        self.channels = channels
        self.out_channels = out_channels or channels
        self.conv = nn.Conv2d(channels, self.out_channels, 3, padding=padding)
        self._pk = None

    def run(self, x):
        if self._pk is None:
            self._pk = ops.pack_conv(self.conv.weight, self.conv.bias)
        if ops.use_dma() and self.channels % 32 == 0:
            x = ops.split_rows(x)
        return ops.conv(x, self._pk, pad=(1, 1), up=(2, 2))


class GEGLU(nn.Module):
    def __init__(self, dim_in, dim_out):
        super().__init__()
        self.proj = nn.Linear(dim_in, dim_out * 2)


class FeedForward(nn.Module):

    def __init__(self, dim, mult=4, dropout=0.0):
        super().__init__()
        self.net = nn.Sequential(GEGLU(dim, dim * mult), nn.Dropout(dropout), nn.Linear(dim * mult, dim))


class CrossAttention(nn.Module):

    def __init__(self, query_dim, context_dim=None, heads=8, dim_head=64, dropout=0.0):
        super().__init__()
        inner = dim_head * heads
        self.heads = heads
        self.dim_head = dim_head
        self.scale = dim_head ** -0.5
        context_dim = query_dim if context_dim is None else context_dim
        self.to_q = nn.Linear(query_dim, inner, bias=False)
        self.to_k = nn.Linear(context_dim, inner, bias=False)
        self.to_v = nn.Linear(context_dim, inner, bias=False)
        self.to_out = nn.Sequential(nn.Linear(inner, query_dim), nn.Dropout(dropout))


class BasicTransformerBlock(nn.Module):

    def __init__(self, dim, n_heads, d_head, dropout=0.0, context_dim=None):
        super().__init__()
        assert d_head == 32, "the HIP attention kernel is specialised for head dim 32 (all AudioLDM2 configs)"
        self.attn1 = CrossAttention(dim, heads=n_heads, dim_head=d_head, dropout=dropout)
        self.ff = FeedForward(dim, dropout=dropout)
        self.attn2 = CrossAttention(dim, context_dim=context_dim, heads=n_heads, dim_head=d_head, dropout=dropout)
        self.norm1 = nn.LayerNorm(dim)
        self.norm2 = nn.LayerNorm(dim)
        self.norm3 = nn.LayerNorm(dim)
        self.heads = n_heads
        self.dim = dim
        self._pk = None
        self._kv = None

    def _context_kv(self, context, pk):
        for c in (self._kv or ()):
            if c[0] is context and c[1] == context._version:
                return c[2]
        kv = ops.linear(context, pk["kv2"])
        if not torch.cuda.is_current_stream_capturing():
            self._kv = [(context, context._version, kv)] + list(self._kv or ())[:1]
        return kv

    def _prepare(self):
        if self._pk is None:
            f = lambda t: t.detach().float().cuda().contiguous()
            a1, a2 = self.attn1, self.attn2
            self._pk = dict(
                ln=[(f(n.weight), f(n.bias)) for n in (self.norm1, self.norm2, self.norm3)],
                qkv1=ops.pack_conv(torch.cat([a1.to_q.weight, a1.to_k.weight, a1.to_v.weight], 0)),
                out1=ops.pack_conv(a1.to_out[0].weight, a1.to_out[0].bias),
                qkv2=ops.pack_conv(torch.cat([a2.to_q.weight, a2.to_k.weight, a2.to_v.weight], 0))
                if a2.to_k.weight.shape[1] == self.dim else None,
                q2=ops.pack_conv(a2.to_q.weight),
                kv2=ops.pack_conv(torch.cat([a2.to_k.weight, a2.to_v.weight], 0)),
                out2=ops.pack_conv(a2.to_out[0].weight, a2.to_out[0].bias),
                ff1=ops.pack_geglu(self.ff.net[0].proj.weight, self.ff.net[0].proj.bias),
                ff2=ops.pack_conv(self.ff.net[2].weight, self.ff.net[2].bias),
            )
        return self._pk

    def run(self, h, context=None, mask=None, want_split=False):
        pk = self._prepare()
        C = self.dim
        so = "only" if (ops.use_dma() and C % 32 == 0) else None
        n = ops.layernorm(h, *pk["ln"][0], split_out=so)
        pre = so is not None and PRESPLIT_ATTENTION and C % 64 == 0 and pk["qkv1"].bias is None
        if pre:
            q, kimg, vtimg = ops.linear_qkv(n, pk["qkv1"], self.heads, h.shape[1])
            a = ops.attention_presplit(q, kimg, vtimg, self.heads, split_out=so)
        else:
            qkv = ops.linear(n, pk["qkv1"])
            a = ops.attention(qkv[:, :, :C], qkv[:, :, C:2 * C], qkv[:, :, 2 * C:], self.heads, split_out=so)
        h = ops.linear(a, pk["out1"], res=h)
        n = ops.layernorm(h, *pk["ln"][1], split_out=so)
        if context is None:
            if pk["qkv2"] is None:
                raise RuntimeError("attn2 was built with a context_dim but no context was provided")
            if pre and pk["qkv2"].bias is None:
                q, kimg, vtimg = ops.linear_qkv(n, pk["qkv2"], self.heads, h.shape[1])
                a = ops.attention_presplit(q, kimg, vtimg, self.heads, split_out=so)
            else:
                qkv = ops.linear(n, pk["qkv2"])
                a = ops.attention(qkv[:, :, :C], qkv[:, :, C:2 * C], qkv[:, :, 2 * C:], self.heads, split_out=so)
        else:
            q = ops.linear(n, pk["q2"])
            kv = self._context_kv(context, pk)
            a = ops.attention(q, kv[:, :, :C], kv[:, :, C:], self.heads, mask=mask, split_out=so)
        h = ops.linear(a, pk["out2"], res=h)
        n = ops.layernorm(h, *pk["ln"][2], split_out=so)
        g = ops.linear_geglu(n, pk["ff1"], split_out=so)
        if want_split and so:
            return ops.linear(g, pk["ff2"], res=h, split_out="also")
        return ops.linear(g, pk["ff2"], res=h)


class SpatialTransformer(nn.Module):

    def __init__(self, in_channels, n_heads, d_head, depth=1, dropout=0.0, context_dim=None):
        super().__init__()
        self.in_channels = in_channels
        inner = n_heads * d_head
        self.norm = nn.GroupNorm(32, in_channels, eps=1e-6, affine=True)
        self.proj_in = nn.Conv2d(in_channels, inner, 1)
        self.transformer_blocks = nn.ModuleList(
            [BasicTransformerBlock(inner, n_heads, d_head, dropout=dropout, context_dim=context_dim)
             for _ in range(depth)])
        self.proj_out = nn.Conv2d(inner, in_channels, 1)
        self._pk = None

    def run(self, x, context=None, mask=None):
        if self._pk is None:
            self._pk = dict(gn=(self.norm.weight.detach().float().cuda().contiguous(),
                                self.norm.bias.detach().float().cuda().contiguous()),
                            pin=ops.pack_conv(self.proj_in.weight, self.proj_in.bias),
                            pout=ops.pack_conv(self.proj_out.weight, self.proj_out.bias))
        pk = self._pk
        B, H, W, C = x.shape
        if ops.use_dma() and C % 32 == 0 and self.proj_in.out_channels % 32 == 0:
            h = ops.conv(ops.gn_split(x, *pk["gn"], groups=32, eps=1e-6), pk["pin"]).view(B, H * W, -1)
            hs = None
            for i, blk in enumerate(self.transformer_blocks):
                r = blk.run(h, context, mask, want_split=i == len(self.transformer_blocks) - 1)
                h, hs = r if isinstance(r, tuple) else (r, None)
            return ops.conv((hs if hs is not None else h).view(B, H, W, -1), pk["pout"], res=x)
        sc, sh = ops.gn_stats(x, *pk["gn"], groups=32, eps=1e-6)
        h = ops.conv(x, pk["pin"], pre=(sc, sh)).view(B, H * W, -1)
        for blk in self.transformer_blocks:
            h = blk.run(h, context, mask)
        return ops.conv(h.view(B, H, W, -1), pk["pout"], res=x)


class TimestepEmbedSequential(nn.Sequential):

    def run(self, x, emb, context_list, mask_list, x2=None, lo=0, hi=None):
        ctxs = [None] + list(context_list)
        masks = [None] + list(mask_list)
        layers = list(self)
        st_id = sum(isinstance(l, SpatialTransformer) for l in layers[:lo])
        for layer in layers[lo:hi]:
            if isinstance(layer, ResBlock):
                x = layer.run(x, emb[layer._emb_slice], x2)
                x2 = None
            elif isinstance(layer, SpatialTransformer):
                if st_id >= len(ctxs):
                    c, m = None, None
                else:
                    c, m = ctxs[st_id], masks[st_id]
                x = layer.run(x, c, m)
                st_id += 1
            elif isinstance(layer, (Downsample, Upsample)):
                x = layer.run(x)
            elif isinstance(layer, _ConvIn):
                x = layer.run(x)
            else:
                raise RuntimeError(f"unexpected layer {type(layer)}")
        assert x2 is None, "skip tensor was not consumed by a ResBlock"
        return x


class _EmbSlices:

    def __init__(self, t):
        self.t = t

    def __getitem__(self, sl):
        return self.t[:, sl]


class _ConvIn(nn.Conv2d):

    _pk = None

    def run(self, x):
        if self._pk is None:
            self._pk = ops.pack_conv(self.weight, self.bias)
        return ops.conv(x, self._pk, pad=(1, 1))


class UNetModel(nn.Module):

    def __init__(self, image_size, in_channels, model_channels, out_channels, num_res_blocks,
                 attention_resolutions, dropout=0, channel_mult=(1, 2, 4, 8), conv_resample=True, dims=2,
                 extra_sa_layer=True, num_classes=None, extra_film_condition_dim=None,
                 use_checkpoint=False, use_fp16=False, num_heads=-1, num_head_channels=-1,
                 num_heads_upsample=-1, use_scale_shift_norm=False, resblock_updown=False,
                 use_new_attention_order=False, use_spatial_transformer=True, transformer_depth=1,
                 context_dim=None, n_embed=None, legacy=True):
        super().__init__()
        if dims != 2 or use_scale_shift_norm or resblock_updown or not use_spatial_transformer \
                or n_embed is not None or num_classes is not None or use_fp16 or not conv_resample:
            raise NotImplementedError("UNetModel(HIP): only the option set used by the AudioLDM2 configs "
                                      "(utils.py:329-343) is implemented")
        if num_heads_upsample == -1:
            num_heads_upsample = num_heads
        assert num_heads != -1 or num_head_channels != -1, "Either num_heads or num_head_channels has to be set"
        self.image_size = image_size
        self.in_channels = in_channels
        self.model_channels = model_channels
        self.out_channels = out_channels
        self.num_res_blocks = num_res_blocks
        self.attention_resolutions = attention_resolutions
        self.channel_mult = channel_mult
        self.extra_film_condition_dim = extra_film_condition_dim
        self.use_extra_film_by_concat = extra_film_condition_dim is not None
        self.dtype = torch.float32
        ted = model_channels * 4
        self.time_embed = nn.Sequential(nn.Linear(model_channels, ted), nn.SiLU(), nn.Linear(ted, ted))
        if self.use_extra_film_by_concat:
            self.film_emb = nn.Linear(extra_film_condition_dim, ted)
        if context_dim is not None and not isinstance(context_dim, (list, tuple)):
            context_dim = [context_dim]
        elif context_dim is None:
            context_dim = [None]
        context_dim = list(context_dim)
        emb_ch = ted * 2 if self.use_extra_film_by_concat else ted

        def transformers(ch):
            if num_head_channels == -1:
                heads, dim_head = num_heads, ch // num_heads
            else:
                heads, dim_head = ch // num_head_channels, num_head_channels
            out = []
            if extra_sa_layer:
                out.append(SpatialTransformer(ch, heads, dim_head, depth=transformer_depth, context_dim=None))
            for cd in context_dim:
                out.append(SpatialTransformer(ch, heads, dim_head, depth=transformer_depth, context_dim=cd))
            return out

        self.input_blocks = nn.ModuleList(
            [TimestepEmbedSequential(_ConvIn(in_channels, model_channels, 3, padding=1))])
        chans = [model_channels]
        ch, ds = model_channels, 1
        for level, mult in enumerate(channel_mult):
            for _ in range(num_res_blocks):
                layers = [ResBlock(ch, emb_ch, dropout, out_channels=mult * model_channels)]
                ch = mult * model_channels
                if ds in attention_resolutions:
                    layers += transformers(ch)
                self.input_blocks.append(TimestepEmbedSequential(*layers))
                chans.append(ch)
            if level != len(channel_mult) - 1:
                self.input_blocks.append(TimestepEmbedSequential(Downsample(ch, True, out_channels=ch)))
                chans.append(ch)
                ds *= 2
        self.middle_block = TimestepEmbedSequential(
            ResBlock(ch, emb_ch, dropout), *transformers(ch), ResBlock(ch, emb_ch, dropout))
        self.output_blocks = nn.ModuleList([])
        for level, mult in list(enumerate(channel_mult))[::-1]:
            for i in range(num_res_blocks + 1):
                ich = chans.pop()
                layers = [ResBlock(ch + ich, emb_ch, dropout, out_channels=model_channels * mult)]
                ch = model_channels * mult
                if ds in attention_resolutions:
                    layers += transformers(ch)
                if level and i == num_res_blocks:
                    layers.append(Upsample(ch, True, out_channels=ch))
                    ds //= 2
                self.output_blocks.append(TimestepEmbedSequential(*layers))
        self.out = nn.Sequential(nn.GroupNorm(32, ch), nn.SiLU(),
                                 nn.Conv2d(model_channels, out_channels, 3, padding=1))
        self._pk = None
        self._graph_cache = {}
        self.register_load_state_dict_post_hook(lambda module, incompatible: module.invalidate_packed())

    def invalidate_packed(self):
        from .ddim import drop_graph_entries
        drop_graph_entries(self._graph_cache)
        for m in self.modules():
            if hasattr(m, "_pk"):
                m._pk = None
            if hasattr(m, "_kv"):
                m._kv = None

    def drop_step_caches(self):
        from .ddim import drop_graph_entries
        drop_graph_entries(self._graph_cache)
        for m in self.modules():
            if hasattr(m, "_kv"):
                m._kv = None

    def collect_context_kv(self, contexts):
        out = []
        for m in self.modules():
            if isinstance(m, BasicTransformerBlock) and m._kv:
                for ctx, _ver, kv in m._kv:
                    if any(ctx is c for c in contexts):
                        out.append((m, ctx, kv))
        return out

    def refresh_context_kv(self, entries):
        n = 0
        for m, ctx, kv in entries:
            pk = m._prepare()
            ops.linear(ctx, pk["kv2"], out=kv)
            m._kv = [(ctx, ctx._version, kv)] + [c for c in (m._kv or ()) if c[2] is not kv][:1]
            n += 1
        return n

    def _prepare(self):
        if self._pk is None:
            f = lambda t: t.detach().float().cuda().contiguous()
            rbs = [m for m in self.modules() if isinstance(m, ResBlock)]
            off = 0
            for m in rbs:
                m._emb_slice = slice(off, off + m.out_channels)
                off += m.out_channels
            self._pk = dict(
                emb_all=ops.pack_conv(torch.cat([m.emb_layers[1].weight for m in rbs], 0),
                                      torch.cat([m.emb_layers[1].bias for m in rbs], 0)),
                te0=ops.pack_conv(self.time_embed[0].weight, self.time_embed[0].bias),
                te2=ops.pack_conv(self.time_embed[2].weight, self.time_embed[2].bias),
                film=ops.pack_conv(self.film_emb.weight, self.film_emb.bias)
                if self.use_extra_film_by_concat else None,
                gn=(f(self.out[0].weight), f(self.out[0].bias)),
                out=ops.pack_conv(self.out[2].weight, self.out[2].bias),
            )
        return self._pk

    def _shared_prefix_end(self, context_list):
        if self.use_extra_film_by_concat:
            return None
        for bi, blk in enumerate(self.input_blocks):
            st = 0
            for li, layer in enumerate(blk):
                if isinstance(layer, SpatialTransformer):
                    if st >= 1 and st - 1 < len(context_list) and context_list[st - 1] is not None:
                        return bi, li
                    st += 1
        return None

    @torch.no_grad()
    def forward(self, x, timesteps=None, y=None, context_list=None, context_attn_mask_list=None, cfg_shared=False, **kwargs):
        assert (y is not None) == self.use_extra_film_by_concat, \
            "must specify y if and only if the model is class-conditional or film embedding conditional"
        if not x.is_cuda:
            raise RuntimeError("UNetModel(HIP) runs on the MI355X only; there is no CPU path")
        pk = self._prepare()
        context_list = [c.float().contiguous() if c is not None else None for c in (context_list or [])]
        mask_list = list(context_attn_mask_list or [])
        div = self._shared_prefix_end(context_list) if cfg_shared else None
        B = x.shape[0]
        if cfg_shared:
            assert timesteps.shape[0] in (B, 2 * B) and all(c is None or c.shape[0] == 2 * B for c in context_list), \
                "cfg_shared: x [B, ...] once, contexts for the 2B rows [uncond ; cond]"
            timesteps = timesteps[:B]
            if div is None:
                x = x.repeat(2, 1, 1, 1)
                timesteps = timesteps.repeat(2)
        t_emb = ops.timestep_embedding(timesteps, self.model_channels)
        emb = ops.linear(ops.linear(t_emb, pk["te0"], act=ACT_SILU), pk["te2"])
        if self.use_extra_film_by_concat:
            emb = torch.cat([emb, ops.linear(y.float().contiguous(), pk["film"])], dim=-1).contiguous()
        emb_rows = ops.linear(emb, pk["emb_all"], pre_act=ACT_SILU)
        emb = _EmbSlices(emb_rows)
        h = ops.nchw_to_nhwc(x.float().contiguous())
        hs = []
        if div is None:
            for module in self.input_blocks:
                h = module.run(h, emb, context_list, mask_list)
                hs.append(h)
        else:
            dup = lambda t: t.repeat(2, *([1] * (t.dim() - 1)))
            emb_half, emb = emb, _EmbSlices(dup(emb_rows))
            for bi, module in enumerate(self.input_blocks):
                if bi < div[0]:
                    h = module.run(h, emb_half, context_list, mask_list)
                elif bi == div[0]:
                    h = module.run(h, emb_half, context_list, mask_list, hi=div[1])
                    h = module.run(dup(h), emb, context_list, mask_list, lo=div[1])
                else:
                    h = module.run(h, emb, context_list, mask_list)
                hs.append(h)
        h = self.middle_block.run(h, emb, context_list, mask_list)
        for module in self.output_blocks:
            skip = hs.pop()
            if skip.shape[0] != h.shape[0]:
                skip = dup(skip)
            h = module.run(h, emb, context_list, mask_list, x2=skip)
        sc, sh = ops.gn_stats(h, *pk["gn"], groups=32, eps=1e-5)
        out = ops.conv(h, pk["out"], pad=(1, 1), pre=(sc, sh), pre_act=ACT_SILU)
        return ops.nhwc_to_nchw(out)
```

include/aldm_hip.h:

```cpp
#ifndef ALDM_HIP_H
#define ALDM_HIP_H

#include <stdint.h>

#ifdef __cplusplus
extern "C" {
#endif

int aldm_version(void);
const char* aldm_last_error(void);

enum {
    ALDM_ACT_NONE = 0,
    ALDM_ACT_SILU = 1,
    ALDM_ACT_LRELU = 2,
    ALDM_ACT_TANH = 3,
    ALDM_ACT_LOGCLAMP = 4,
    ALDM_ACT_GELU = 5,
    ALDM_ACT_GELU_TANH = 6
};

enum { ALDM_EPI_PLAIN = 0, ALDM_EPI_GEGLU = 1, ALDM_EPI_QKV = 2 };

enum {
    ALDM_B_PACKED = 0,
    ALDM_B_NT = 1
};

enum { ALDM_MMA_F32 = 0, ALDM_MMA_BF16X6 = 1 };

typedef struct aldm_igemm_desc {
    const float* x1;
    const float* x2;
    int32_t C1, C2;
    int32_t pix1, pix2;
    int32_t B, H, W;
    int32_t up_h, up_w;
    int32_t KH, KW, SH, SW, PH, PW, DH, DW;
    int32_t OH, OW;
    const float* pre_scale;
    const float* pre_shift;
    int32_t pre_act;
    float pre_slope;
    const float* w;
    int32_t b_mode;
    int32_t ldb;
    int32_t K, N;
    const float* bias;
    const float* rowbias;
    const float* res;
    float* out;
    int32_t ldo;
    int32_t act;
    float act_slope;
    float alpha;
    int32_t accumulate;
    int32_t out_mul, out_off, out_len;
    int32_t batch;
    int64_t stride_x, stride_w, stride_o;
    int32_t rowbias_ld;
    int32_t epi_mode;
    float* ws;
    int64_t ws_floats;
    int32_t hint_bm, hint_bn, hint_splits;
    int32_t hint_kgroups;
    const void* w_split;
    int32_t hint_mma;
    int32_t hint_stages;
    const void* a_split;
    void* out_split;
    int32_t out_split_c;
    int32_t split_parts;
    int32_t out_split_act;
    float out_split_slope;
    void* k_split;
    void* vt_split;
    int32_t qkv_c;
    int32_t qkv_rows;
    int32_t a_fmt;
    float acc_scale;
    int32_t out_split_parts;
    int32_t out_split_fmt;
    float out_split_scale;
    float vt_scale;
} aldm_igemm_desc;

int aldm_igemm(const aldm_igemm_desc* d, void* stream);
int64_t aldm_igemm_ws_floats(const aldm_igemm_desc* d);
enum { ALDM_FMT_BF16 = 0, ALDM_FMT_F16 = 1 };
int aldm_igemm_plan(const aldm_igemm_desc* d, int* bm, int* bn, int64_t* flops, int* splits, int* kgroups,
                    int* mma);
int aldm_igemm_plan_stages(const aldm_igemm_desc* d);
void aldm_igemm_force(int bm, int bn, int splits, int kgroups);
void aldm_igemm_force_stages(int stages);
int aldm_igemm_wave8_mask(int mask);
int aldm_igemm_mma(int mode);
#ifdef ALDM_TEST_HOOKS
int aldm_debug_drop_product(int on);
#endif
int64_t aldm_split_bytes(int K, int N);
int aldm_pack_split_bf16(const float* packed, void* dst, int K, int N, void* stream);
int64_t aldm_split_bytes_parts(int K, int N, int parts);
int aldm_pack_split_bf16_parts(const float* packed, void* dst, int K, int N, int parts, void* stream);
int aldm_pack_split_f16(const float* packed, void* dst, int K, int N, float scale, void* stream);

int64_t aldm_split_image_bytes(int64_t rows, int C, int parts);
int aldm_split_rows(const float* x1, const float* x2, int C1, int C2, int64_t rows, int P, const float* scale,
                    const float* shift, int act, void* dst, void* dst_raw, int parts, void* stream);
int aldm_split_rows_act(const float* x1, const float* x2, int C1, int C2, int64_t rows, int P, const float* scale,
                        const float* shift, int act, float slope, void* dst, void* dst_raw, int parts, void* stream);
int aldm_split_rows_f16(const float* x1, const float* x2, int C1, int C2, int64_t rows, int P, const float* scale,
                        const float* shift, int act, float slope, void* dst, void* dst_raw, int raw_parts, float f16_scale,
                        void* stream);

int aldm_pack_weight(const float* src, float* dst, int N, int Cin, int KH, int KW,
                     int transposed, int phase, int stride, void* stream);
int aldm_pack_kn(const float* src, float* dst, int K, int N, int lds, int batch,
                 int64_t stride_src, int64_t stride_dst, void* stream);

int aldm_groupnorm_stats(const float* x1, const float* x2, int B, int P, int C1, int C2,
                         int G, float eps, const float* gamma, const float* beta,
                         float* scale, float* shift, float* ws, void* stream);
int64_t aldm_gn_ws_floats(int B, int P, int C, int G);
int aldm_groupnorm_split(const float* x1, const float* x2, int B, int P, int C1, int C2, int G, float eps,
                         const float* gamma, const float* beta, int act, float* scale, float* shift, float* ws,
                         void* dst, void* dst_raw, int parts, void* stream);
int aldm_groupnorm_split_f16(const float* x1, const float* x2, int B, int P, int C1, int C2, int G, float eps,
                             const float* gamma, const float* beta, int act, float* scale, float* shift, float* ws,
                             void* dst, void* dst_raw, int raw_parts, float f16_scale, void* stream);
int aldm_layernorm(const float* x, float* y, int M, int C, const float* gamma,
                   const float* beta, float eps, void* stream);
int aldm_layernorm_split(const float* x, float* y, void* y_split, int M, int C, const float* gamma,
                         const float* beta, float eps, int parts, void* stream);
int aldm_layernorm_split_f16(const float* x, float* y, void* y_split, int M, int C, const float* gamma,
                             const float* beta, float eps, float f16_scale, void* stream);

int aldm_attention_d32(const float* q, const float* k, const float* v, float* out,
                       int B, int heads, int Lq, int Lk, int ldq, int ldk, int ldv, int ldo,
                       const float* mask, float scale, void* stream);
int aldm_attention_d32_split(const float* q, const float* k, const float* v, float* out, void* out_split,
                             int parts, int B, int heads, int Lq, int Lk, int ldq, int ldk, int ldv, int ldo,
                             const float* mask, float scale, void* stream);
int aldm_attention_d32_presplit(const float* q, const void* k_split, const void* vt_split, float* out, void* out_split,
                                int parts, int B, int heads, int Lq, int Lk, int ldq, int ldo, float scale, void* stream);
int aldm_vt_regroup(const void* src, void* dst, int B, int L, int heads, int parts, void* stream);
int aldm_attention_mma(int mode);
int aldm_attention_sched(int sched);
int aldm_attention_d32_presplit_f16(const float* q, const void* k_split, const void* vt_split, float* out, void* out_split,
                                    int out_parts, float out_scale, int B, int heads, int Lq, int Lk, int ldq, int ldo,
                                    float scale, float q_scale, float k_scale, float v_scale, void* stream);
int aldm_rel_attention(const float* q, const float* k, const float* v, float* out, int B, int heads, int T, int d,
                       int ldq, int ldk, int ldv, int ldo, const float* emb_k, const float* emb_v, int window,
                       const float* mask, void* stream);
int aldm_rowscale_add(const float* x, const float* s, const float* res, float* y, int64_t rows, int C, int divide,
                      void* stream);
int aldm_rmsnorm(const float* x, float* y, int M, int C, const float* weight, float eps, void* stream);
int aldm_softmax_rows_bias(const float* x, float* y, int B, int heads, int q_rows, int N, float scale, const float* bias,
                           const float* keymask, void* stream);
int aldm_softmax_rows(const float* x, float* y, int64_t M, int N, float scale, void* stream);
int aldm_softmax_rows_masked(const float* x, float* y, int B, int heads, int q_rows, int N, float scale,
                             const float* keymask, int q_pos0, void* stream);

int aldm_decode_linear(const float* x, int ldx, int M, int K, const float* w_kn, int N, const float* bias,
                       const float* ln_gamma, const float* ln_beta, float ln_eps, int act, const float* res, int ldr,
                       float* y, int ldy, void* stream);
int aldm_decode_attention(const float* qkv, int ldq, const int64_t* pos, float* k_cache, float* v_cache, const float* keymask,
                          int B, int heads, int n_tot, float scale, float* out, int ldo, void* stream);
int aldm_decode_gemv_slices(int K, int N);
int aldm_decode_gemv(const float* x, int ldx, int xparts, int64_t xstride, const float* xbias, int xact, int M, int K,
                     const float* w_kn, int N, float* ypart, void* stream);
int aldm_decode_reduce_ln(const float* part, int nparts, int64_t pstride, int ldp, const float* bias, const int64_t* bias_row,
                          const float* res, int ldr, int M, int N, float* h_out, int ldh, const float* ln_gamma,
                          const float* ln_beta, float ln_eps, float* xn, int ldn, float* xn2, int ldn2, void* stream);
int aldm_decode_attention_parts(const float* qkv_part, int ldq, int qparts, int64_t qstride, const float* qbias,
                                const int64_t* pos, float* k_cache, float* v_cache, const float* keymask, int B, int heads,
                                int n_tot, float scale, float* out, int ldo, void* stream);

int aldm_geglu(const float* x, float* y, int64_t M, int C, void* stream);
int aldm_timestep_embedding(const float* t, float* out, int B, int dim, float max_period,
                            void* stream);
int aldm_nchw_to_nhwc(const float* x, float* y, int B, int C, int HW, int rep, void* stream);
int aldm_nhwc_to_nchw(const float* x, float* y, int B, int C, int HW, void* stream);
int aldm_ddim_step(const float* x, const float* eps, const float* noise, const float* coef,
                   float* x_prev, float* pred_x0, int64_t n, void* stream);
int aldm_ddim_step_indexed(float* x, const float* eps, const float* noise_tab, const float* coef_tab,
                           const int* step_idx, float* pred_x0, int64_t n, int coef_ld, void* stream);
int aldm_plms_first_step(const float* x, const float* e_t, const float* e_next, const float* coef_row, float* x_out,
                         float* pred_x0, float* hist, int64_t n, void* stream);
int aldm_plms_step_indexed(float* x, const float* eps, float* hist, const float* coef_tab, const int* step_idx,
                           float* pred_x0, int64_t n, int coef_ld, void* stream);
int aldm_step_advance(int* step_idx, const float* t_tab, float* t_cur, int nt, int steps, void* stream);
int aldm_ddpm_step(const float* x, const float* eps, const float* noise, const float* coef,
                   float* x_prev, int64_t n, void* stream);
int aldm_inpaint_blend(const float* x0, const float* qnoise, const float* mask, const float* coef,
                       float* x, int64_t n, void* stream);
int aldm_axpby(const float* a, const float* b, float* y, float alpha, float beta, int64_t n,
               void* stream);
int aldm_reflect_pad_1d(const float* x, float* y, int B, int T, int pad, int ld_out,
                        void* stream);
int aldm_mag_phase(const float* spec, float* mag, float* phase, int64_t M, int F, int ld_spec,
                   int ld_mag, void* stream);

int aldm_row_l2norm(const float* x, float* out, int64_t M, int F, int ld, void* stream);

int aldm_resample_sinc(const float* x, const float* kernel, float* y, int B, int T, int Tout, int down, int up, int taps,
                       int width, void* stream);
int aldm_power_spec(const float* spec, float* out, int64_t M, int F, int ld_spec, int ld_out, void* stream);
int aldm_col_affine(const float* x, const float* scale, const float* shift, float* y, int64_t rows, int C, void* stream);
int aldm_bicubic_patchify(const float* x, float* out, int B, int T, int mel, int S, int p, void* stream);
int aldm_token_mean(const float* x, float* y, int B, int L, int C, void* stream);
int aldm_row_cosine(const float* a, const float* b, float* out, int M, int C, float eps, void* stream);

#ifdef __cplusplus
}
#endif
#endif
```

Measured before the change: 19.32 audio-s/s.

## Prefetch next GEMM/conv weights into cache from within norm kernels

Norm kernels (groupnorm partial/fused and layernorm) now take a list of up to four memory regions, the weights of the following conv or linear layers, and touch every 128-byte line of them spread across all threads. The loaded values are kept live through an empty asm so the compiler cannot drop the loads. The aim is to warm L2/LLC so the next weight-heavy GEMM starts with its weights cached, hiding the cold weight fetch behind the memory-bound norm. In exchange the norm kernels issue extra loads and hold extra registers, which adds bandwidth and latency to them, and the benefit depends on the weights staying resident in cache until the next kernel runs.

```diff
diff --git a/audioldm2_amd/csrc/api.hip b/audioldm2_amd/csrc/api.hip
--- a/audioldm2_amd/csrc/api.hip
+++ b/audioldm2_amd/csrc/api.hip
@@ -11,5 +11,5 @@
 }
 }
 
-extern "C" int aldm_version(void) { return 11; }
+extern "C" int aldm_version(void) { return 12; }
 extern "C" const char* aldm_last_error(void) { return aldm::g_err; }
diff --git a/audioldm2_amd/csrc/norm.hip b/audioldm2_amd/csrc/norm.hip
--- a/audioldm2_amd/csrc/norm.hip
+++ b/audioldm2_amd/csrc/norm.hip
@@ -1,7 +1,15 @@
 #include <stdlib.h>
 #include "igemm_epilogue.h"
+#include "prefetch.h"
 
 namespace aldm {
+
+static thread_local PrefetchList g_next_prefetch = {};
+
+struct PfTaken {
+    PrefetchList list;
+    PfTaken() : list(g_next_prefetch) { g_next_prefetch.count = 0; }
+};
 
 constexpr int GN_ITERS = 16;
 constexpr int GN_UNROLL = 8;
@@ -27,7 +35,7 @@
                                                          const float* __restrict__ gamma,
                                                          const float* __restrict__ beta,
                                                          float* __restrict__ scale, float* __restrict__ shift, int gpb,
-                                                         char* __restrict__ dst = nullptr, char* __restrict__ dst_raw = nullptr,
+                                                         PrefetchList pf, char* __restrict__ dst = nullptr, char* __restrict__ dst_raw = nullptr,
                                                          int parts = 3, int act = ALDM_ACT_NONE, int raw_parts = 3,
                                                          float f16_scale = 0.f) {
     const int C = C1 + C2;
@@ -45,6 +53,7 @@
     __shared__ double gacc[64][3];
     if (tid < 64) gacc[tid][0] = gacc[tid][1] = gacc[tid][2] = 0.0;
     __syncthreads();
+    PfHeld held = {};
     for (int cp = 0; cp < npass; ++cp) {
         const int c4 = c4_lo + cp * cols + tx;
         GnPart part = {0.f, 0.f, 0.f};
@@ -89,6 +98,7 @@
             part.mean = pivot + md;
             part.m2 = fmaxf(ss - s * md, 0.f);
         }
+        if (cp == 0) held = prefetch_regions(pf, (int64_t)blockIdx.y * gridDim.x + blockIdx.x, (int64_t)gridDim.x * gridDim.y);
         if constexpr (FUSED) {
             __shared__ double wred[4][3];
             const int mygl = (c4 - c4_lo) / Cg4;
@@ -207,6 +217,7 @@
         w[1] = gacc[tid][1];
         w[2] = gacc[tid][2];
     }
+    prefetch_retire(held);
 }
 
 __global__ __launch_bounds__(256) void gn_finalize_kernel(const float* __restrict__ ws, int chunks,
@@ -262,10 +273,14 @@
                                                         float* __restrict__ y, int M, int C,
                                                         const float* __restrict__ gamma,
                                                         const float* __restrict__ beta, float eps,
-                                                        void* __restrict__ y_split, int parts, float f16_scale) {
+                                                        void* __restrict__ y_split, int parts, float f16_scale,
+                                                        PrefetchList pf) {
     const int lane = threadIdx.x & 63;
     const int row0 = (blockIdx.x * 4 + (threadIdx.x >> 6)) * R;
-    if (row0 >= M) return;
+    if (row0 >= M) {
+        prefetch_retire(prefetch_regions(pf, blockIdx.x, gridDim.x));
+        return;
+    }
     const int C4 = C >> 2;
     f32x4 v[R][MAXV];
 #pragma unroll
@@ -284,6 +299,7 @@
         ga[i] = *reinterpret_cast<const f32x4*>(gamma + 4 * c4);
         be[i] = RMS ? f32x4{0.f, 0.f, 0.f, 0.f} : *reinterpret_cast<const f32x4*>(beta + 4 * c4);
     }
+    const PfHeld held = prefetch_regions(pf, blockIdx.x, gridDim.x);
     float mean[R], rstd[R];
 #pragma unroll
     for (int r = 0; r < R; ++r) {
@@ -332,6 +348,7 @@
             }
         }
     }
+    prefetch_retire(held);
 }
 
 template <bool MASKED, bool BIASED = false>
@@ -396,6 +413,15 @@
 
 using namespace aldm;
 
+extern "C" int aldm_norm_prefetch(const aldm_prefetch_list* list) {
+    g_next_prefetch.count = 0;
+    if (list == nullptr) return 0;
+    ALDM_CHECK(list->count >= 0 && list->count <= ALDM_PREFETCH_MAX_REGIONS, "aldm_norm_prefetch: count %d not in 0..%d", list->count,
+               ALDM_PREFETCH_MAX_REGIONS);
+    g_next_prefetch = *list;
+    return 0;
+}
+
 extern "C" int64_t aldm_gn_ws_floats(int B, int P, int C, int G) {
     int cols, rows, chunk_px, chunks;
     gn_geometry(P, C, &cols, &rows, &chunk_px, &chunks);
@@ -410,7 +436,8 @@
 
 static int groupnorm_launch(const float* x1, const float* x2, int B, int P, int C1, int C2, int G, float eps,
                             const float* gamma, const float* beta, float* scale, float* shift, float* ws, void* dst,
-                            void* dst_raw, int parts, int act, void* stream, int raw_parts = 0, float f16_scale = 0.f) {
+                            void* dst_raw, int parts, int act, void* stream, const PrefetchList& pf, int raw_parts = 0,
+                            float f16_scale = 0.f) {
     if (raw_parts == 0) raw_parts = parts;
     if (!x2) C2 = 0;
     const int C = C1 + C2;
@@ -438,16 +465,16 @@
         }();
         if (dst && fuse_split && slab % 8 == 0 && slab <= 256 && C1 % 8 == 0) {
             hipLaunchKernelGGL(gn_partial_kernel<true>, dim3(gs, B), dim3(256), 0, st, x1, x2, P, C1, C2, G, fcols, frows, P, ws,
-                               eps, gamma, beta, scale, shift, gpb, reinterpret_cast<char*>(dst),
+                               eps, gamma, beta, scale, shift, gpb, pf, reinterpret_cast<char*>(dst),
                                reinterpret_cast<char*>(dst_raw), parts, act, raw_parts, f16_scale);
             ALDM_LAUNCH_CHECK("aldm_groupnorm_split");
             return 0;
         }
         hipLaunchKernelGGL(gn_partial_kernel<true>, dim3(gs, B), dim3(256), 0, st, x1, x2, P, C1, C2, G, fcols,
-                           frows, P, ws, eps, gamma, beta, scale, shift, gpb, nullptr, nullptr, 3, ALDM_ACT_NONE);
+                           frows, P, ws, eps, gamma, beta, scale, shift, gpb, pf, nullptr, nullptr, 3, ALDM_ACT_NONE);
     } else {
         hipLaunchKernelGGL(gn_partial_kernel<false>, dim3(chunks, B), dim3(256), 0, st, x1, x2, P, C1, C2, G,
-                           cols, rows, chunk_px, ws, eps, gamma, beta, scale, shift, G);
+                           cols, rows, chunk_px, ws, eps, gamma, beta, scale, shift, G, pf);
         hipLaunchKernelGGL(gn_finalize_kernel, dim3(B), dim3(256), 0, st, ws, chunks, P, C, G, eps, gamma,
                            beta, scale, shift);
     }
@@ -463,36 +490,40 @@
 extern "C" int aldm_groupnorm_stats(const float* x1, const float* x2, int B, int P, int C1, int C2,
                                     int G, float eps, const float* gamma, const float* beta,
                                     float* scale, float* shift, float* ws, void* stream) {
+    const PfTaken pf;
     return groupnorm_launch(x1, x2, B, P, C1, C2, G, eps, gamma, beta, scale, shift, ws, nullptr, nullptr, 3, ALDM_ACT_NONE,
-                            stream);
+                            stream, pf.list);
 }
 
 extern "C" int aldm_groupnorm_split(const float* x1, const float* x2, int B, int P, int C1, int C2, int G, float eps,
                                     const float* gamma, const float* beta, int act, float* scale, float* shift, float* ws,
                                     void* dst, void* dst_raw, int parts, void* stream) {
+    const PfTaken pf;
     if (!x2) C2 = 0;
     ALDM_CHECK(dst != nullptr && (parts == 2 || parts == 3) && (C1 + C2) % 32 == 0 && C1 % 8 == 0 && C2 % 8 == 0,
                "aldm_groupnorm_split: need dst, parts 2|3, (C1+C2) %% 32 == 0, C1 %% 8 == 0 (C1=%d C2=%d)", C1, C2);
     ALDM_CHECK(act == ALDM_ACT_NONE || act == ALDM_ACT_SILU, "aldm_groupnorm_split: activation %d not supported", act);
     ALDM_CHECK(((reinterpret_cast<uintptr_t>(dst) | reinterpret_cast<uintptr_t>(dst_raw)) & 15) == 0,
                "aldm_groupnorm_split: split images must be 16-byte aligned");
-    return groupnorm_launch(x1, x2, B, P, C1, C2, G, eps, gamma, beta, scale, shift, ws, dst, dst_raw, parts, act, stream);
+    return groupnorm_launch(x1, x2, B, P, C1, C2, G, eps, gamma, beta, scale, shift, ws, dst, dst_raw, parts, act, stream, pf.list);
 }
 
 extern "C" int aldm_groupnorm_split_f16(const float* x1, const float* x2, int B, int P, int C1, int C2, int G, float eps,
                                         const float* gamma, const float* beta, int act, float* scale, float* shift, float* ws,
                                         void* dst, void* dst_raw, int raw_parts, float f16_scale, void* stream) {
+    const PfTaken pf;
     if (!x2) C2 = 0;
     ALDM_CHECK(dst != nullptr && f16_scale > 0.0f && (raw_parts == 2 || raw_parts == 3) && (C1 + C2) % 32 == 0 && C1 % 8 == 0 && C2 % 8 == 0,
                "aldm_groupnorm_split_f16: need dst, f16_scale > 0, raw_parts 2|3, (C1+C2) %% 32 == 0, C1 %% 8 == 0 (C1=%d C2=%d)", C1, C2);
     ALDM_CHECK(act == ALDM_ACT_NONE || act == ALDM_ACT_SILU, "aldm_groupnorm_split_f16: activation %d not supported", act);
     ALDM_CHECK(((reinterpret_cast<uintptr_t>(dst) | reinterpret_cast<uintptr_t>(dst_raw)) & 15) == 0,
                "aldm_groupnorm_split_f16: split images must be 16-byte aligned");
-    return groupnorm_launch(x1, x2, B, P, C1, C2, G, eps, gamma, beta, scale, shift, ws, dst, dst_raw, 2, act, stream, raw_parts, f16_scale);
+    return groupnorm_launch(x1, x2, B, P, C1, C2, G, eps, gamma, beta, scale, shift, ws, dst, dst_raw, 2, act, stream, pf.list, raw_parts, f16_scale);
 }
 
 static int layernorm_launch(const float* x, float* y, void* y_split, int parts, int M, int C, const float* gamma,
-                            const float* beta, float eps, void* stream, const char* name, bool rms = false, float f16_scale = 0.f) {
+                            const float* beta, float eps, void* stream, const char* name, const PrefetchList& pf, bool rms = false,
+                            float f16_scale = 0.f) {
     ALDM_CHECK(parts == 2 || parts == 3, "%s: parts must be 2 or 3", name);
     ALDM_CHECK(x && (y || y_split) && gamma && (beta || rms), "%s: null pointer", name);
     ALDM_CHECK(C % 4 == 0 && C <= 256 * LN_MAXV, "%s: C=%d must be a multiple of 4 and <= %d", name, C, 256 * LN_MAXV);
@@ -503,10 +534,10 @@
     do {                                                                                                            \
         if (rms)                                                                                                    \
             hipLaunchKernelGGL((layernorm_kernel<V_, R_, true>), dim3(cdiv(M, 4 * R_)), dim3(256), 0, st, x, y, M, C, \
-                               gamma, beta, eps, y_split, parts, f16_scale);                                        \
+                               gamma, beta, eps, y_split, parts, f16_scale, pf);                                    \
         else                                                                                                        \
             hipLaunchKernelGGL((layernorm_kernel<V_, R_, false>), dim3(cdiv(M, 4 * R_)), dim3(256), 0, st, x, y, M, \
-                               C, gamma, beta, eps, y_split, parts, f16_scale);                                     \
+                               C, gamma, beta, eps, y_split, parts, f16_scale, pf);                                 \
     } while (0)
     const int nv = cdiv(C / 4, 64);
     static const int env_r = [] {
@@ -530,22 +561,26 @@
 
 extern "C" int aldm_layernorm(const float* x, float* y, int M, int C, const float* gamma,
                               const float* beta, float eps, void* stream) {
-    return layernorm_launch(x, y, nullptr, 3, M, C, gamma, beta, eps, stream, "aldm_layernorm");
+    const PfTaken pf;
+    return layernorm_launch(x, y, nullptr, 3, M, C, gamma, beta, eps, stream, "aldm_layernorm", pf.list);
 }
 
 extern "C" int aldm_layernorm_split(const float* x, float* y, void* y_split, int M, int C, const float* gamma,
                                     const float* beta, float eps, int parts, void* stream) {
-    return layernorm_launch(x, y, y_split, parts, M, C, gamma, beta, eps, stream, "aldm_layernorm_split");
+    const PfTaken pf;
+    return layernorm_launch(x, y, y_split, parts, M, C, gamma, beta, eps, stream, "aldm_layernorm_split", pf.list);
 }
 
 extern "C" int aldm_layernorm_split_f16(const float* x, float* y, void* y_split, int M, int C, const float* gamma,
                                         const float* beta, float eps, float f16_scale, void* stream) {
+    const PfTaken pf;
     ALDM_CHECK(y_split != nullptr && f16_scale > 0.0f, "aldm_layernorm_split_f16: need y_split and f16_scale > 0");
-    return layernorm_launch(x, y, y_split, 2, M, C, gamma, beta, eps, stream, "aldm_layernorm_split_f16", false, f16_scale);
+    return layernorm_launch(x, y, y_split, 2, M, C, gamma, beta, eps, stream, "aldm_layernorm_split_f16", pf.list, false, f16_scale);
 }
 
 extern "C" int aldm_rmsnorm(const float* x, float* y, int M, int C, const float* weight, float eps, void* stream) {
-    return layernorm_launch(x, y, nullptr, 3, M, C, weight, nullptr, eps, stream, "aldm_rmsnorm", true);
+    const PfTaken pf;
+    return layernorm_launch(x, y, nullptr, 3, M, C, weight, nullptr, eps, stream, "aldm_rmsnorm", pf.list, true);
 }
 
 extern "C" int aldm_softmax_rows(const float* x, float* y, int64_t M, int N, float scale,
diff --git a/audioldm2_amd/csrc/prefetch.h b/audioldm2_amd/csrc/prefetch.h
--- /dev/null
+++ b/audioldm2_amd/csrc/prefetch.h
@@ -0,0 +1,81 @@
+#pragma once
+#include <stdint.h>
+#include "../../include/aldm_hip.h"
+
+#if defined(__HIPCC__) || defined(__CUDACC__)
+#define ALDM_HD __host__ __device__ inline
+#else
+#define ALDM_HD inline
+#endif
+
+namespace aldm {
+
+constexpr int PF_LINE = 128;
+constexpr int PF_HELD = 4;
+
+typedef aldm_prefetch_list PrefetchList;
+
+ALDM_HD int64_t pf_region_lines(const void* ptr, int64_t bytes) {
+    return (ptr != nullptr && bytes >= 4) ? (int64_t)((uint64_t)(bytes - 4) / PF_LINE) + 1 : 0;
+}
+
+ALDM_HD int64_t pf_total_lines(const PrefetchList& l) {
+    int64_t n = 0;
+#pragma unroll
+    for (int r = 0; r < ALDM_PREFETCH_MAX_REGIONS; ++r) n += r < l.count ? pf_region_lines(l.ptr[r], l.bytes[r]) : 0;
+    return n;
+}
+
+ALDM_HD int64_t pf_line_index(int64_t block, int64_t nblocks, int thread, int nthreads, int64_t k) {
+    return (k * nblocks + block) * nthreads + thread;
+}
+
+ALDM_HD const uint32_t* pf_line_addr(const PrefetchList& l, int64_t idx, int* region = nullptr) {
+    const char* base = nullptr;
+    int64_t line = 0;
+    int reg = -1;
+#pragma unroll
+    for (int r = 0; r < ALDM_PREFETCH_MAX_REGIONS; ++r) {
+        const int64_t n = r < l.count ? pf_region_lines(l.ptr[r], l.bytes[r]) : 0;
+        const bool hit = reg < 0 && idx >= 0 && idx < n;
+        base = hit ? static_cast<const char*>(l.ptr[r]) : base;
+        line = hit ? idx : line;
+        reg = hit ? r : reg;
+        idx -= n;
+    }
+    if (region) *region = reg;
+    return reg < 0 ? nullptr : reinterpret_cast<const uint32_t*>(base + line * PF_LINE);
+}
+
+#if defined(__HIPCC__)
+struct PfHeld {
+    uint32_t v[PF_HELD];
+};
+
+__device__ __forceinline__ void prefetch_retire(const PfHeld& h) {
+#pragma unroll
+    for (int u = 0; u < PF_HELD; ++u) asm volatile("" ::"v"(h.v[u]));
+}
+
+__device__ __forceinline__ PfHeld prefetch_regions(const PrefetchList& l, int64_t block, int64_t nblocks) {
+    PfHeld h;
+#pragma unroll
+    for (int u = 0; u < PF_HELD; ++u) h.v[u] = 0u;
+    const int64_t total = pf_total_lines(l);
+    if (total > 0) {
+        const int nthreads = (int)blockDim.x;
+        const int64_t T = nblocks * nthreads;
+        for (int64_t k0 = 0; k0 * T < total; k0 += PF_HELD) {
+            if (k0 > 0) prefetch_retire(h);
+#pragma unroll
+            for (int u = 0; u < PF_HELD; ++u) {
+                const int64_t idx = pf_line_index(block, nblocks, (int)threadIdx.x, nthreads, k0 + u);
+                if (idx < total) h.v[u] = *pf_line_addr(l, idx);
+            }
+        }
+    }
+    return h;
+}
+#endif
+
+}
diff --git a/audioldm2_amd/lib.py b/audioldm2_amd/lib.py
--- a/audioldm2_amd/lib.py
+++ b/audioldm2_amd/lib.py
@@ -5,7 +5,7 @@
 
 _HERE = os.path.dirname(os.path.abspath(__file__))
 LIB_PATH = os.environ.get("ALDM_LIB_PATH") or os.path.join(_HERE, "libaldm_hip.so")
-ABI_VERSION = 11
+ABI_VERSION = 12
 
 ACT_NONE, ACT_SILU, ACT_LRELU, ACT_TANH, ACT_LOGCLAMP, ACT_GELU, ACT_GELU_TANH = range(7)
 B_PACKED, B_NT = 0, 1
@@ -47,8 +47,17 @@
     ]
 
 
+PREFETCH_MAX_REGIONS = 4
+
+
+class PrefetchList(C.Structure):
+
+    _fields_ = [("ptr", C.c_void_p * PREFETCH_MAX_REGIONS), ("bytes", C.c_int64 * PREFETCH_MAX_REGIONS), ("count", C.c_int32)]
+
+
 _SIGS = {
     "aldm_version": (C.c_int, []),
+    "aldm_norm_prefetch": (C.c_int, [C.POINTER(PrefetchList)]),
     "aldm_last_error": (C.c_char_p, []),
     "aldm_igemm": (C.c_int, [C.POINTER(IgemmDesc), C.c_void_p]),
     "aldm_igemm_plan": (C.c_int, [C.POINTER(IgemmDesc), C.POINTER(C.c_int), C.POINTER(C.c_int),
diff --git a/audioldm2_amd/ops.py b/audioldm2_amd/ops.py
--- a/audioldm2_amd/ops.py
+++ b/audioldm2_amd/ops.py
@@ -274,6 +274,54 @@
 
 def use_dma() -> bool:
     return DMA_MODE and MMA_MODE in ("bf16x6", "bf16x3", "f16x3")
+
+
+WEIGHT_PREFETCH = os.environ.get("ALDM_WEIGHT_PREFETCH", "0") != "0"
+PREFETCH_MAX_BYTES = int(os.environ.get("ALDM_PREFETCH_MAX_BYTES", str(2 << 20)))
+
+
+def set_weight_prefetch(on: bool, max_bytes: Optional[int] = None) -> Tuple[bool, int]:
+    global WEIGHT_PREFETCH, PREFETCH_MAX_BYTES
+    prev = (WEIGHT_PREFETCH, PREFETCH_MAX_BYTES)
+    WEIGHT_PREFETCH = bool(on)
+    if max_bytes is not None:
+        PREFETCH_MAX_BYTES = int(max_bytes)
+    return prev
+
+
+def prefetch_regions(weights: Optional[Sequence[Optional["Packed"]]]) -> List[Tuple[int, int]]:
+    out = []
+    if not WEIGHT_PREFETCH or not weights:
+        return out
+    for pw in weights:
+        if pw is None:
+            continue
+        if MMA_MODE == "f32":
+            img = pw.data
+        elif MMA_MODE == "f16x3" and pw.split16 is not None:
+            img = pw.split16
+        elif MMA_MODE == "bf16x3" and pw.split2 is not None:
+            img = pw.split2
+        else:
+            img = pw.split
+        if img is None:
+            continue
+        nbytes = min(img.numel() * img.element_size(), PREFETCH_MAX_BYTES)
+        if nbytes >= 4 and len(out) < _l.PREFETCH_MAX_REGIONS:
+            out.append((img.data_ptr(), nbytes))
+    return out
+
+
+def _arm_prefetch(lib, weights) -> None:
+    regs = prefetch_regions(weights)
+    if not regs:
+        return
+    pl = _l.PrefetchList()
+    pl.count = len(regs)
+    for i, (ptr, nbytes) in enumerate(regs):
+        pl.ptr[i] = ptr
+        pl.bytes[i] = nbytes
+    _l.check(lib.aldm_norm_prefetch(C.byref(pl)), "norm_prefetch")
 
 
 def split_rows(x: torch.Tensor, x2: Optional[torch.Tensor] = None, pre=None, act: int = ACT_NONE,
@@ -817,7 +865,7 @@
 
 
 def gn_stats(x: torch.Tensor, gamma: torch.Tensor, beta: torch.Tensor, *, groups: int = 32,
-             eps: float = 1e-5, x2: Optional[torch.Tensor] = None):
+             eps: float = 1e-5, x2: Optional[torch.Tensor] = None, prefetch=None):
     _chk(x, "gn.x")
     B = x.shape[0]
     C1 = x.shape[-1]
@@ -831,6 +879,7 @@
     nws = lib.aldm_gn_ws_floats(B, P, Cc, groups)
     ws = torch.empty(nws, device=x.device, dtype=torch.float32)
     ss = torch.empty((2, B, Cc), device=x.device, dtype=torch.float32)
+    _arm_prefetch(lib, prefetch)
     _l.check(lib.aldm_groupnorm_stats(x.data_ptr(), _p(x2), B, P, C1, C2, groups, eps,
                                       gamma.data_ptr(), beta.data_ptr(), ss[0].data_ptr(),
                                       ss[1].data_ptr(), ws.data_ptr(), _stream()), "groupnorm_stats")
@@ -838,7 +887,7 @@
 
 
 def gn_split(x: torch.Tensor, gamma: torch.Tensor, beta: torch.Tensor, *, groups: int = 32, eps: float = 1e-5,
-             x2: Optional[torch.Tensor] = None, act: int = ACT_NONE, want_raw: bool = False):
+             x2: Optional[torch.Tensor] = None, act: int = ACT_NONE, want_raw: bool = False, prefetch=None):
     _chk(x, "gn_split.x")
     B = x.shape[0]
     C1 = x.shape[-1]
@@ -856,11 +905,13 @@
     raw = SplitT.empty(shape, x.device) if want_raw else None
     if f16_mode():
         dst = SplitT.empty(shape, x.device, f16_scale=_norm_f16_scale(gamma, beta, (Cc // groups) * P))
+        _arm_prefetch(lib, prefetch)
         _l.check(lib.aldm_groupnorm_split_f16(x.data_ptr(), _p(x2), B, P, C1, C2, groups, eps, gamma.data_ptr(), beta.data_ptr(), act,
                                               ss[0].data_ptr(), ss[1].data_ptr(), ws.data_ptr(), dst.data_ptr(),
                                               None if raw is None else raw.data_ptr(), 3, dst.scale, _stream()), "groupnorm_split_f16")
         return (dst, raw) if want_raw else dst
     dst = SplitT.empty(shape, x.device)
+    _arm_prefetch(lib, prefetch)
     _l.check(lib.aldm_groupnorm_split(x.data_ptr(), _p(x2), B, P, C1, C2, groups, eps, gamma.data_ptr(), beta.data_ptr(), act,
                                       ss[0].data_ptr(), ss[1].data_ptr(), ws.data_ptr(), dst.data_ptr(),
                                       None if raw is None else raw.data_ptr(), dst.parts, _stream()), "groupnorm_split")
@@ -868,12 +919,13 @@
 
 
 def layernorm(x: torch.Tensor, gamma: torch.Tensor, beta: torch.Tensor, eps: float = 1e-5,
-              split_out: Optional[str] = None):
+              split_out: Optional[str] = None, prefetch=None):
     _chk(x, "ln.x")
     Cc = x.shape[-1]
     M = x.numel() // Cc
     y = None if split_out == "only" else torch.empty_like(x)
     if not split_out:
+        _arm_prefetch(_l.load(), prefetch)
         _l.check(_l.load().aldm_layernorm(x.data_ptr(), y.data_ptr(), M, Cc, gamma.data_ptr(),
                                           beta.data_ptr(), eps, _stream()), "layernorm")
         return y
@@ -881,10 +933,12 @@
         so = SplitT.empty(x.shape, x.device, f16_scale=_norm_f16_scale(gamma, beta, Cc))
         so.rn = _row_norm_bound(gamma, beta, Cc)
         so.rt = _row_norm_typical(gamma, beta)
+        _arm_prefetch(_l.load(), prefetch)
         _l.check(_l.load().aldm_layernorm_split_f16(x.data_ptr(), _p(y), so.data_ptr(), M, Cc, gamma.data_ptr(), beta.data_ptr(), eps,
                                                     so.scale, _stream()), "layernorm_split_f16")
         return so if split_out == "only" else (y, so)
     so = SplitT.empty(x.shape, x.device)
+    _arm_prefetch(_l.load(), prefetch)
     _l.check(_l.load().aldm_layernorm_split(x.data_ptr(), _p(y), so.data_ptr(), M, Cc, gamma.data_ptr(),
                                             beta.data_ptr(), eps, so.parts, _stream()), "layernorm_split")
     return so if split_out == "only" else (y, so)
diff --git a/audioldm2_amd/unet.py b/audioldm2_amd/unet.py
--- a/audioldm2_amd/unet.py
+++ b/audioldm2_amd/unet.py
@@ -51,16 +51,17 @@
         if ops.use_dma() and self.channels % 32 == 0 and x.shape[-1] % 8 == 0 and c2 % 8 == 0:
             if pk["skip"] is None:
                 assert x2 is None
-                a1, skip = ops.gn_split(x, *pk["gn1"], groups=32, eps=1e-5, act=ACT_SILU), x
+                a1, skip = ops.gn_split(x, *pk["gn1"], groups=32, eps=1e-5, act=ACT_SILU, prefetch=(pk["conv1"],)), x
             else:
-                a1, araw = ops.gn_split(x, *pk["gn1"], groups=32, eps=1e-5, x2=x2, act=ACT_SILU, want_raw=True)
+                a1, araw = ops.gn_split(x, *pk["gn1"], groups=32, eps=1e-5, x2=x2, act=ACT_SILU, want_raw=True,
+                                        prefetch=(pk["skip"], pk["conv1"]))
                 skip = ops.conv(araw, pk["skip"])
             h = ops.conv(a1, pk["conv1"], pad=(1, 1), rowbias=e)
-            a2 = ops.gn_split(h, *pk["gn2"], groups=32, eps=1e-5, act=ACT_SILU)
+            a2 = ops.gn_split(h, *pk["gn2"], groups=32, eps=1e-5, act=ACT_SILU, prefetch=(pk["conv2"],))
             return ops.conv(a2, pk["conv2"], pad=(1, 1), res=skip)
-        sc, sh = ops.gn_stats(x, *pk["gn1"], groups=32, eps=1e-5, x2=x2)
+        sc, sh = ops.gn_stats(x, *pk["gn1"], groups=32, eps=1e-5, x2=x2, prefetch=(pk["conv1"],))
         h = ops.conv(x, pk["conv1"], x2=x2, pad=(1, 1), pre=(sc, sh), pre_act=ACT_SILU, rowbias=e)
-        sc2, sh2 = ops.gn_stats(h, *pk["gn2"], groups=32, eps=1e-5)
+        sc2, sh2 = ops.gn_stats(h, *pk["gn2"], groups=32, eps=1e-5, prefetch=(pk["skip"], pk["conv2"]))
         if pk["skip"] is None:
             assert x2 is None
             skip = x
@@ -176,11 +177,11 @@
             )
         return self._pk
 
-    def run(self, h, context=None, mask=None, want_split=False):
+    def run(self, h, context=None, mask=None, want_split=False, pout=None):
         pk = self._prepare()
         C = self.dim
         so = "only" if (ops.use_dma() and C % 32 == 0) else None
-        n = ops.layernorm(h, *pk["ln"][0], split_out=so)
+        n = ops.layernorm(h, *pk["ln"][0], split_out=so, prefetch=(pk["qkv1"], pk["out1"]))
         pre = so is not None and PRESPLIT_ATTENTION and C % 64 == 0 and pk["qkv1"].bias is None
         if pre:
             q, kimg, vtimg = ops.linear_qkv(n, pk["qkv1"], self.heads, h.shape[1])
@@ -189,7 +190,8 @@
             qkv = ops.linear(n, pk["qkv1"])
             a = ops.attention(qkv[:, :, :C], qkv[:, :, C:2 * C], qkv[:, :, 2 * C:], self.heads, split_out=so)
         h = ops.linear(a, pk["out1"], res=h)
-        n = ops.layernorm(h, *pk["ln"][1], split_out=so)
+        n = ops.layernorm(h, *pk["ln"][1], split_out=so,
+                          prefetch=(pk["qkv2"] if context is None else pk["q2"], pk["out2"]))
         if context is None:
             if pk["qkv2"] is None:
                 raise RuntimeError("attn2 was built with a context_dim but no context was provided")
@@ -204,7 +206,7 @@
             kv = self._context_kv(context, pk)
             a = ops.attention(q, kv[:, :, :C], kv[:, :, C:], self.heads, mask=mask, split_out=so)
         h = ops.linear(a, pk["out2"], res=h)
-        n = ops.layernorm(h, *pk["ln"][2], split_out=so)
+        n = ops.layernorm(h, *pk["ln"][2], split_out=so, prefetch=(pk["ff1"], pk["ff2"], pout))
         g = ops.linear_geglu(n, pk["ff1"], split_out=so)
         if want_split and so:
             return ops.linear(g, pk["ff2"], res=h, split_out="also")
@@ -234,13 +236,14 @@
         pk = self._pk
         B, H, W, C = x.shape
         if ops.use_dma() and C % 32 == 0 and self.proj_in.out_channels % 32 == 0:
-            h = ops.conv(ops.gn_split(x, *pk["gn"], groups=32, eps=1e-6), pk["pin"]).view(B, H * W, -1)
+            h = ops.conv(ops.gn_split(x, *pk["gn"], groups=32, eps=1e-6, prefetch=(pk["pin"],)), pk["pin"]).view(B, H * W, -1)
             hs = None
             for i, blk in enumerate(self.transformer_blocks):
-                r = blk.run(h, context, mask, want_split=i == len(self.transformer_blocks) - 1)
+                last = i == len(self.transformer_blocks) - 1
+                r = blk.run(h, context, mask, want_split=last, pout=pk["pout"] if last else None)
                 h, hs = r if isinstance(r, tuple) else (r, None)
             return ops.conv((hs if hs is not None else h).view(B, H, W, -1), pk["pout"], res=x)
-        sc, sh = ops.gn_stats(x, *pk["gn"], groups=32, eps=1e-6)
+        sc, sh = ops.gn_stats(x, *pk["gn"], groups=32, eps=1e-6, prefetch=(pk["pin"],))
         h = ops.conv(x, pk["pin"], pre=(sc, sh)).view(B, H * W, -1)
         for blk in self.transformer_blocks:
             h = blk.run(h, context, mask)
diff --git a/include/aldm_hip.h b/include/aldm_hip.h
--- a/include/aldm_hip.h
+++ b/include/aldm_hip.h
@@ -135,6 +135,14 @@
 int aldm_layernorm_split_f16(const float* x, float* y, void* y_split, int M, int C, const float* gamma,
                              const float* beta, float eps, float f16_scale, void* stream);
 
+#define ALDM_PREFETCH_MAX_REGIONS 4
+typedef struct aldm_prefetch_list {
+    const void* ptr[ALDM_PREFETCH_MAX_REGIONS];
+    int64_t bytes[ALDM_PREFETCH_MAX_REGIONS];
+    int32_t count;
+} aldm_prefetch_list;
+int aldm_norm_prefetch(const aldm_prefetch_list* list);
+
 int aldm_attention_d32(const float* q, const float* k, const float* v, float* out,
                        int B, int heads, int Lq, int Lk, int ldq, int ldk, int ldv, int ldo,
                        const float* mask, float scale, void* stream);
```

Result: no change. 19.20 audio-s/s (-0.6%).
